# Ezreal11/EaBNet

Measured on AMD Instinct MI355X. Metric: enhanced frames/sec (16 kHz, 8-mic) at 1/2/4/8 MI355X; RTF per utterance, higher is better.
Workload: dtype f32; 1 GPU; BASELINE configs[1]/[2]: batch of 16 four-second 8-mic 16 kHz utterances per GPU, wave -> STFT+compress -> EaBNet.forward, inference, full hand-written HIP path; batch_per_gpu=16, global_batch=16, mics=8, frames_per_utt=401, freq_bins=161, parallelism=dp1 (independent shards, no collective), pipeline_depth=3

## Files before the change

### eabnet_amd/_lib.py

```python
from __future__ import annotations

import ctypes as C
import os
from typing import Optional

_HERE = os.path.dirname(os.path.abspath(__file__))
LIB_PATH = os.path.join(_HERE, "lib", "libeabnet_hip.so")
ABI_VERSION = 10
MAX_TAPS = 16
_fp = C.POINTER(C.c_float)


class TimeWindow(C.Structure):
    _fields_ = [("pos", C.c_void_p), ("count", C.c_int32), ("lens", C.c_void_p)]


class ConvDesc(C.Structure):
    _fields_ = [
        ("src0", C.c_void_p), ("src1", C.c_void_p), ("xf0", C.c_void_p), ("xf1", C.c_void_p),
        ("slope0", C.c_void_p), ("slope1", C.c_void_p),
        ("C0", C.c_int32), ("C1", C.c_int32), ("xf_mode", C.c_int32),
        ("w", C.c_void_p), ("bias", C.c_void_p),
        ("N", C.c_int32), ("Kpad", C.c_int32),
        ("B", C.c_int32), ("T", C.c_int32), ("Fin", C.c_int32), ("Fout", C.c_int32),
        ("No", C.c_int32), ("ostride", C.c_int32), ("ophase", C.c_int32), ("istride", C.c_int32),
        ("ntaps", C.c_int32), ("dt", C.c_int32 * MAX_TAPS), ("ioff", C.c_int32 * MAX_TAPS),
        ("epi", C.c_int32),
        ("aux", C.c_void_p), ("dst", C.c_void_p), ("dst_acc", C.c_void_p),
        ("Cout", C.c_int32),
        ("stats", C.c_void_p), ("nsets", C.c_int32),
        ("stat_slope0", C.c_void_p), ("stat_slope1", C.c_void_p),
        ("stat_tiles", C.c_int32), ("stat_tile0", C.c_int32), ("bm", C.c_int32),
        ("fin_stats", C.c_void_p), ("fin_gamma0", C.c_void_p), ("fin_beta0", C.c_void_p),
        ("fin_gamma1", C.c_void_p), ("fin_beta1", C.c_void_p),
        ("fin_tiles", C.c_int32), ("fin_nsets", C.c_int32), ("fin_count", C.c_int32), ("fin_eps", C.c_float),
        ("precision", C.c_int32), ("korder", C.c_int32),
        ("win", TimeWindow),
        ("fz_counter", C.c_void_p), ("fz_gamma0", C.c_void_p), ("fz_beta0", C.c_void_p), ("fz_xf0", C.c_void_p),
        ("fz_gamma1", C.c_void_p), ("fz_beta1", C.c_void_p), ("fz_xf1", C.c_void_p), ("fz_eps", C.c_float),
        ("glu_dump", C.c_void_p),
        ("ph1_w", C.c_void_p), ("ph1_No", C.c_int32), ("ph1_ophase", C.c_int32), ("ph1_ntaps", C.c_int32), ("ph1_Kpad", C.c_int32),
        ("ph1_dt", C.c_int32 * MAX_TAPS), ("ph1_ioff", C.c_int32 * MAX_TAPS),
        ("f2_w", C.c_void_p), ("f2_dst", C.c_void_p), ("f2_stats", C.c_void_p), ("f2_stat_slope0", C.c_void_p),
        ("f2_stat_slope1", C.c_void_p), ("f2_N", C.c_int32), ("f2_nsets", C.c_int32), ("f2_stat_tiles", C.c_int32),
        ("p2_mask1", C.c_int32), ("src_bf16", C.c_int32),
    ]


class WgradDesc(C.Structure):
    _fields_ = [
        ("dz", C.c_void_p), ("src0", C.c_void_p), ("src1", C.c_void_p), ("dw", C.c_void_p), ("dbias", C.c_void_p),
        ("N", C.c_int32), ("C0", C.c_int32), ("C1", C.c_int32), ("Kpad", C.c_int32),
        ("B", C.c_int32), ("T", C.c_int32), ("Fin", C.c_int32), ("Fz", C.c_int32), ("No", C.c_int32),
        ("ostride", C.c_int32), ("ophase", C.c_int32), ("istride", C.c_int32),
        ("ntaps", C.c_int32), ("dt", C.c_int32 * MAX_TAPS), ("ioff", C.c_int32 * MAX_TAPS),
        ("rows_per_wg", C.c_int32), ("precision", C.c_int32), ("bf16_mask", C.c_int32),
    ]


class Op(C.Structure):
    _fields_ = [("kind", C.c_int32), ("i", C.c_int32 * 8), ("f", C.c_float * 2), ("p", C.c_void_p * 12),
                ("win", TimeWindow), ("conv", ConvDesc), ("wgrad", WgradDesc)]


class ShiftDesc(C.Structure):
    _fields_ = [("ptr", C.c_void_p), ("row_floats", C.c_int32), ("rows", C.c_int32)]


class EabError(RuntimeError):
    pass


_SIGS = {
    "eab_abi_version": (C.c_int, []),
    "eab_error_string": (C.c_char_p, [C.c_int]),
    "eab_stft_compress_f32": (C.c_int, [C.c_void_p] * 4 + [C.c_int] * 6 + [C.c_void_p]),
    "eab_stft_compress_lens_f32": (C.c_int, [C.c_void_p] * 5 + [C.c_int] * 6 + [C.c_void_p]),
    "eab_stft_frames_f32": (C.c_int, [C.c_void_p] * 2 + [C.c_int] * 5 + [C.c_void_p]),
    "eab_filter_sum_f32": (C.c_int, [C.c_void_p] * 3 + [C.c_int] * 4 + [C.c_void_p]),
    "eab_istft_f32": (C.c_int, [C.c_void_p] * 4 + [C.c_int] * 4 + [C.c_void_p]),
    "eab_istft_lens_f32": (C.c_int, [C.c_void_p] * 5 + [C.c_int] * 4 + [C.c_void_p]),
    "eab_norm_act_win_f32": (C.c_int, [C.c_void_p] * 7 + [C.c_int] * 4 + [TimeWindow, C.c_void_p]),
    "eab_lstm64_stream_f32": (C.c_int, [C.c_void_p] * 3 + [C.c_float] + [C.c_void_p] * 4 + [C.c_int] * 4
                              + [TimeWindow, C.c_void_p]),
    "eab_bfw_filter_sum_win_f32": (C.c_int, [C.c_void_p] * 6 + [C.c_int] * 4 + [TimeWindow, C.c_void_p]),
    "eab_mlp_bfw_filter_sum_f32": (C.c_int, [C.c_void_p] * 8 + [C.c_int] * 4 + [TimeWindow, C.c_void_p]),
    "eab_zero_rows_f32": (C.c_int, [C.c_void_p] + [C.c_int] * 3 + [TimeWindow, C.c_void_p]),
    "eab_shift_rows_f32": (C.c_int, [C.c_void_p] + [C.c_int] * 5 + [C.c_void_p]),
    "eab_com_mag_mse_loss_f32": (C.c_int, [C.c_void_p] * 3 + [C.c_int] * 3 + [C.c_void_p, C.c_int, C.c_void_p, C.c_void_p,
                                            C.c_void_p]),
    "eab_energy_ratios_f32": (C.c_int, [C.c_void_p, C.c_longlong, C.c_int] * 3 + [C.c_void_p, C.c_int, C.c_void_p, C.c_int,
                                        C.c_void_p, C.c_void_p]),
    "eab_com_mag_mse_loss_lens_f32": (C.c_int, [C.c_void_p] * 3 + [C.c_int] * 4 + [C.c_void_p, C.c_int, C.c_void_p, C.c_void_p]),
    "eab_gag_pack_f32": (C.c_int, [C.c_void_p] * 4 + [C.c_int] * 4 + [TimeWindow, C.c_void_p]),
    "eab_gag_crm_f32": (C.c_int, [C.c_void_p] * 6 + [C.c_int] * 6 + [TimeWindow, C.c_void_p]),
    "eab_gag_crm_bwd_f32": (C.c_int, [C.c_void_p] * 9 + [C.c_int] * 6 + [C.c_void_p]),
    "eab_conv_tiles": (C.c_int, [C.c_int] * 3),
    "eab_conv_f32": (C.c_int, [C.POINTER(ConvDesc), C.c_void_p]),
    "eab_train_cln_bwd_f32": (C.c_int, [C.c_void_p] * 11 + [C.c_int] * 5 + [C.c_void_p]),
    "eab_conv_st_chain_plan": (C.c_int, [C.POINTER(ConvDesc), C.c_int, C.POINTER(C.c_int), C.POINTER(C.c_int), C.POINTER(C.c_int)]),
    "eab_conv_st_chain_run": (C.c_int, [C.c_void_p, C.c_void_p, C.c_int, C.c_int, C.c_int, C.c_int, C.c_void_p]),
    "eab_conv_bf16": (C.c_int, [C.POINTER(ConvDesc), C.c_void_p]),
    "eab_lstm64_bf16": (C.c_int, [C.c_void_p] * 3 + [C.c_float] + [C.c_void_p] * 3 + [C.c_int] * 3 + [C.c_void_p]),
    "eab_in_finalize_f32": (C.c_int, [C.c_void_p] + [C.c_int] * 5 + [C.c_float] + [C.c_void_p] * 6 + [C.c_void_p]),
    "eab_norm_act_f32": (C.c_int, [C.c_void_p] * 7 + [C.c_int] * 3 + [C.c_void_p]),
    "eab_lstm64_f32": (C.c_int, [C.c_void_p] * 3 + [C.c_float] + [C.c_void_p] * 3 + [C.c_int] * 3 + [C.c_void_p]),
    "eab_lstm64_prec_f32": (C.c_int, [C.c_void_p] * 3 + [C.c_float] + [C.c_void_p] * 3 + [C.c_int] * 4 + [C.c_void_p]),
    "eab_bfw_filter_sum_f32": (C.c_int, [C.c_void_p] * 6 + [C.c_int] * 4 + [C.c_void_p]),
    "eab_run_program": (C.c_int, [C.POINTER(Op), C.c_int, C.c_void_p]),
    "eab_sizeof_conv_desc": (C.c_int, []),
    "eab_sizeof_op": (C.c_int, []),
    "eab_sizeof_wgrad_desc": (C.c_int, []),
    "eab_gather_f32": (C.c_int, [C.c_void_p] * 4 + [C.c_longlong, C.c_void_p]),
    "eab_train_in_stats_f32": (C.c_int, [C.c_void_p] * 2 + [C.c_int] * 3 + [C.c_float] + [C.c_void_p] * 4 + [C.c_void_p]),
    "eab_train_in1d_f32": (C.c_int, [C.c_void_p] * 2 + [C.c_int] * 3 + [C.c_float] + [C.c_void_p] * 5 + [C.c_void_p]),
    "eab_train_in1d_multi_f32": (C.c_int, [C.c_void_p] * 2 + [C.c_int] * 4 + [C.c_float] + [C.c_void_p] * 5 + [C.c_void_p]),
    "eab_train_norm_bwd_multi_f32": (C.c_int, [C.c_void_p] * 12 + [C.c_int] * 3 + [C.c_void_p]),
    "eab_in_finalize_mr_f32": (C.c_int, [C.c_void_p] + [C.c_int] * 5 + [C.c_float] + [C.c_void_p] * 8 + [C.c_void_p]),
    "eab_train_norm_act_f32": (C.c_int, [C.c_void_p] * 5 + [C.c_int] * 4 + [C.c_void_p]),
    "eab_train_norm_bwd_f32": (C.c_int, [C.c_void_p] * 12 + [C.c_int] * 4 + [C.c_void_p]),
    "eab_glu_bwd_f32": (C.c_int, [C.c_void_p] * 3 + [C.c_longlong, C.c_int, C.c_void_p]),
    "eab_glu_bwd_ex_f32": (C.c_int, [C.c_void_p] * 3 + [C.c_longlong, C.c_int, C.c_int, C.c_void_p]),
    "eab_gate_fwd_f32": (C.c_int, [C.c_void_p] * 3 + [C.c_longlong, C.c_void_p]),
    "eab_gate_bwd_f32": (C.c_int, [C.c_void_p] * 5 + [C.c_longlong, C.c_void_p]),
    "eab_add_f32": (C.c_int, [C.c_void_p] * 3 + [C.c_longlong, C.c_void_p]),
    "eab_copy_f32": (C.c_int, [C.c_void_p] * 2 + [C.c_longlong, C.c_void_p]),
    "eab_relu_bwd_f32": (C.c_int, [C.c_void_p] * 3 + [C.c_longlong, C.c_void_p]),
    "eab_colsum_f32": (C.c_int, [C.c_void_p] * 2 + [C.c_longlong, C.c_int, C.c_void_p]),
    "eab_filter_sum_bwd_f32": (C.c_int, [C.c_void_p] * 3 + [C.c_int] * 5 + [C.c_void_p]),
    "eab_filter_sum_ld_f32": (C.c_int, [C.c_void_p] * 3 + [C.c_int] * 5 + [C.c_void_p]),
    "eab_layernorm64_fwd_f32": (C.c_int, [C.c_void_p] * 3 + [C.c_float] + [C.c_void_p] * 2 + [C.c_longlong, C.c_void_p]),
    "eab_layernorm64_bwd_f32": (C.c_int, [C.c_void_p] * 7 + [C.c_longlong, C.c_void_p]),
    "eab_lstm64_train_fwd_f32": (C.c_int, [C.c_void_p] * 5 + [C.c_int] * 3 + [C.c_void_p]),
    "eab_lstm64_bwd_f32": (C.c_int, [C.c_void_p] * 4 + [C.c_int] * 3 + [C.c_void_p]),
    "eab_lstm64_train_fwd_prec_f32": (C.c_int, [C.c_void_p] * 5 + [C.c_int] * 4 + [C.c_void_p]),
    "eab_lstm64_bwd_prec_f32": (C.c_int, [C.c_void_p] * 4 + [C.c_int] * 4 + [C.c_void_p]),
    "eab_wgrad_f32": (C.c_int, [C.POINTER(WgradDesc), C.c_void_p]),
    "eab_wgrad_batchable": (C.c_int, [C.c_void_p, C.c_int, C.c_int]),
    "eab_wgrad_batch_f32": (C.c_int, [C.c_void_p, C.c_int, C.c_int, C.c_void_p]),
    "eab_cln_stats_f32": (C.c_int, [C.c_void_p] * 2 + [C.c_int] * 4 + [C.c_float] + [C.c_void_p] * 3 + [TimeWindow, C.c_void_p]),
    "eab_cln_apply_f32": (C.c_int, [C.c_void_p] * 7 + [C.c_int] * 5 + [TimeWindow, C.c_void_p]),
    "eab_cln_step_f32": (C.c_int, [C.c_void_p] * 10 + [C.c_int] * 5 + [C.c_float, TimeWindow, C.c_void_p]),
    "eab_gate_rows_f32": (C.c_int, [C.c_void_p] * 3 + [C.c_int] * 3 + [TimeWindow, C.c_void_p]),
}
EXPORTS = tuple(_SIGS)

_lib: Optional[C.CDLL] = None


def load() -> C.CDLL:
    global _lib
    if _lib is not None:
        return _lib
    if not os.path.exists(LIB_PATH):
        raise EabError(
            f"{LIB_PATH} not found: build it with `python -c 'import __graft_entry__ as g; g.build()'` "
            "(or `make -C eabnet_amd/csrc`). eabnet_amd has no CPU fallback by design.")
    lib = C.CDLL(LIB_PATH)
    for name, (res, args) in _SIGS.items():
        try:
            fn = getattr(lib, name)
        except AttributeError as e:
            raise EabError(f"{LIB_PATH} does not export {name}") from e
        fn.restype, fn.argtypes = res, args
    if lib.eab_abi_version() != ABI_VERSION:
        raise EabError(f"ABI mismatch: library {lib.eab_abi_version()} != binding {ABI_VERSION}")
    if lib.eab_sizeof_conv_desc() != C.sizeof(ConvDesc) or lib.eab_sizeof_op() != C.sizeof(Op) \
            or lib.eab_sizeof_wgrad_desc() != C.sizeof(WgradDesc):
        raise EabError("struct layout mismatch between include/eabnet_hip.h and eabnet_amd/_lib.py")
    _lib = lib
    return lib


def check(code: int, what: str = "") -> None:
    if code != 0:
        msg = load().eab_error_string(code).decode()
        raise EabError(f"{what or 'libeabnet_hip'} failed with code {code}: {msg}")
```

### eabnet_amd/csrc/lstm.hip

```cpp
#include "common.h"
#include <cstdlib>
#include <type_traits>

#define LS_H 64
#define LS_SEQ 16
#define LS_LD (LS_H + 4)

__device__ __forceinline__ float ls_sigmoid(float x) { return __builtin_amdgcn_rcpf(1.0f + __expf(-x)); }
__device__ __forceinline__ float ls_tanh(float x) { return fmaf(2.0f, ls_sigmoid(2.0f * x), -1.0f); }

__device__ __forceinline__ float ls_row_sum(float v) {
    auto dpp = [](float x, auto ctrl) {
        return __builtin_bit_cast(float, __builtin_amdgcn_update_dpp(0, __builtin_bit_cast(int, x), decltype(ctrl)::value, 0xF, 0xF, true));
    };
    v += dpp(v, std::integral_constant<int, 0xB1>{});
    v += dpp(v, std::integral_constant<int, 0x4E>{});
    v += dpp(v, std::integral_constant<int, 0x141>{});
    v += dpp(v, std::integral_constant<int, 0x140>{});
    return v;
}

typedef unsigned int u32x4 __attribute__((ext_vector_type(4)));
#define LS_OOB 0x80000000u

template <bool LN, bool DUMP>
__global__ __launch_bounds__(256) void lstm64_kernel(const float* __restrict__ x, const float* __restrict__ ln_g,
                                                     const float* __restrict__ ln_b, float ln_eps,
                                                     const float* __restrict__ wcat, const float* __restrict__ bias,
                                                     float* __restrict__ h_out, int T, int F, int S,
                                                     const int* __restrict__ t_pos, int t_count,
                                                     float* __restrict__ c_state, float* __restrict__ gates,
                                                     const int* __restrict__ lens = nullptr) {
    __shared__ __attribute__((aligned(16))) float xs[2][LS_SEQ * LS_LD];
    __shared__ __attribute__((aligned(16))) float hs[2][LS_SEQ * LS_LD];
    const int tid = threadIdx.x, lane = tid & 63, wave = tid >> 6;
    const int ln = lane & 15, lk = lane >> 4;
    const int s0 = blockIdx.x * LS_SEQ;
    const int t_lo = t_pos ? *t_pos : 0;
    int t_hi = t_pos ? (t_lo + t_count < T ? t_lo + t_count : T) : T;
    if (lens) t_hi = min(t_hi, eab_max_len(lens, s0, LS_SEQ, S, F));

    float wx[4][16], wh[4][16];
    float bia[4];
#pragma unroll
    for (int g = 0; g < 4; ++g) {
        const int row = g * LS_H + wave * 16 + ln;
        bia[g] = bias[row];
#pragma unroll
        for (int j = 0; j < 4; ++j) {
            const f32x4 vx = *reinterpret_cast<const f32x4*>(&wcat[(size_t)row * 128 + 16 * j + 4 * lk]);
            const f32x4 vh = *reinterpret_cast<const f32x4*>(&wcat[(size_t)row * 128 + 64 + 16 * j + 4 * lk]);
#pragma unroll
            for (int s = 0; s < 4; ++s) {
                wx[g][4 * j + s] = vx[s];
                wh[g][4 * j + s] = vh[s];
            }
        }
    }

    const int ls = tid >> 4, lc = (tid & 15) * 4;
    const int sg = s0 + ls;
    const bool sv = sg < S;
    const int sb = sv ? sg / F : 0, sf = sv ? sg - sb * F : 0;
    const unsigned total_bytes = (unsigned)S * (unsigned)T * (LS_H * 4u);
    const __amdgpu_buffer_rsrc_t rx = __builtin_amdgcn_make_buffer_rsrc(const_cast<float*>(x), 0, total_bytes, 0x00020000);
    const __amdgpu_buffer_rsrc_t rh = __builtin_amdgcn_make_buffer_rsrc(h_out, 0, total_bytes, 0x00020000);
    const unsigned seq_off = (unsigned)((((size_t)sb * T * F + sf) * LS_H + lc) * 4);
    const unsigned t_stride = (unsigned)F * LS_H * 4u;
    f32x4 g4 = {1.f, 1.f, 1.f, 1.f}, b4 = {0.f, 0.f, 0.f, 0.f};
    if (LN) {
        g4 = *reinterpret_cast<const f32x4*>(ln_g + lc);
        b4 = *reinterpret_cast<const f32x4*>(ln_b + lc);
    }

    auto load_x = [&](int t) -> f32x4 {
        const unsigned off = (sv && t < t_hi) ? seq_off + (unsigned)t * t_stride : LS_OOB;
        return __builtin_bit_cast(f32x4, __builtin_amdgcn_raw_buffer_load_b128(rx, off, 0, 0));
    };
    auto norm_store = [&](f32x4 v, int buf) {
        if (LN) {
            const float mean = ls_row_sum((v[0] + v[1]) + (v[2] + v[3])) * (1.0f / 64.0f);
            f32x4 dlt = {v[0] - mean, v[1] - mean, v[2] - mean, v[3] - mean};
            const float q = ls_row_sum((dlt[0] * dlt[0] + dlt[1] * dlt[1]) + (dlt[2] * dlt[2] + dlt[3] * dlt[3]));
            const float rstd = 1.0f / sqrtf(q * (1.0f / 64.0f) + ln_eps);
#pragma unroll
            for (int j = 0; j < 4; ++j) v[j] = dlt[j] * rstd * g4[j] + b4[j];
        }
        *reinterpret_cast<f32x4*>(&xs[buf][ls * LS_LD + lc]) = v;
    };
    auto frags = [&](const float* tile, f32x4 (&a)[4]) {
        const float* arow = tile + ln * LS_LD + 4 * lk;
#pragma unroll
        for (int j = 0; j < 4; ++j) a[j] = *reinterpret_cast<const f32x4*>(arow + 16 * j);
    };
    auto mma = [&](const f32x4 (&a)[4], const float (&w)[4][16], f32x4 (&acc)[4], auto j0, auto j1) {
#pragma unroll
        for (int j = decltype(j0)::value; j < decltype(j1)::value; ++j)
#pragma unroll
            for (int s = 0; s < 4; ++s)
#pragma unroll
                for (int g = 0; g < 4; ++g)
                    acc[g] = __builtin_amdgcn_mfma_f32_16x16x4f32(a[j][s], w[g][4 * j + s], acc[g], 0, 0, 0);
    };
    using I0 = std::integral_constant<int, 0>;
    using I2 = std::integral_constant<int, 2>;
    using I4 = std::integral_constant<int, 4>;

    *reinterpret_cast<f32x4*>(&hs[0][ls * LS_LD + lc]) = __builtin_bit_cast(
        f32x4, __builtin_amdgcn_raw_buffer_load_b128(rh, (sv && t_lo > 0) ? seq_off + (unsigned)(t_lo - 1) * t_stride : LS_OOB, 0, 0));
    norm_store(load_x(t_lo), 0);
    norm_store(load_x(t_lo + 1), 1);
    const int u = wave * 16 + ln;
    float cst[4] = {0.f, 0.f, 0.f, 0.f};
    if (c_state && t_lo > 0) {
#pragma unroll
        for (int r = 0; r < 4; ++r)
            if (s0 + 4 * lk + r < S) cst[r] = c_state[(size_t)(s0 + 4 * lk + r) * LS_H + u];
    }
    __syncthreads();
    f32x4 accx[4], hf[4], xf[4];
#pragma unroll
    for (int g = 0; g < 4; ++g) accx[g] = f32x4{bia[g], bia[g], bia[g], bia[g]};
    frags(xs[0], xf);
    mma(xf, wx, accx, I0{}, I4{});
    frags(hs[0], hf);
    asm volatile("s_waitcnt lgkmcnt(0)\n\ts_barrier" ::: "memory");
    f32x4 xq = load_x(t_lo + 2), xr = load_x(t_lo + 3);

    for (int t = t_lo; t < t_hi; ++t) {
        const int cur = (t - t_lo) & 1, nxt = cur ^ 1;
        const f32x4 xn = load_x(t + 4);

        f32x4 acc[4];
#pragma unroll
        for (int g = 0; g < 4; ++g) acc[g] = accx[g];
        mma(hf, wh, acc, I0{}, I4{});
        norm_store(xq, cur);
        frags(xs[nxt], xf);
        if (LN) {
#pragma unroll
            for (int i = 0; i < 16; ++i) {
                __builtin_amdgcn_sched_group_barrier(0x008, 4, 0);
                __builtin_amdgcn_sched_group_barrier(0x002, 6, 0);
            }
        }
        __builtin_amdgcn_sched_barrier(0);

#pragma unroll
        for (int g = 0; g < 4; ++g) accx[g] = f32x4{bia[g], bia[g], bia[g], bia[g]};
        float ev[16], hval[4];
#pragma unroll
        for (int i = 0; i < 32; ++i) {
            {
                const int j = i >> 4, k = (i >> 2) & 3, g = i & 3;
                accx[g] = __builtin_amdgcn_mfma_f32_16x16x4f32(xf[j][k], wx[g][4 * j + k], accx[g], 0, 0, 0);
            }
            if (i < 8) {
#pragma unroll
                for (int n = 2 * i; n < 2 * i + 2; ++n) {
                    const float v = acc[n >> 2][n & 3];
                    ev[n] = __expf((n >> 2) == 2 ? -2.0f * v : -v);
                }
            } else if (i < 16) {
#pragma unroll
                for (int n = 2 * (i - 8); n < 2 * (i - 8) + 2; ++n) {
                    const float sg = __builtin_amdgcn_rcpf(1.0f + ev[n]);
                    ev[n] = (n >> 2) == 2 ? fmaf(2.0f, sg, -1.0f) : sg;
                }
            } else if (i < 20) {
                const int r = i - 16;
                cst[r] = fmaf(ev[4 + r], cst[r], ev[r] * ev[8 + r]);
                hval[r] = __expf(-2.0f * cst[r]);
            } else if (i < 24) {
                const int r = i - 20;
                hval[r] = ev[12 + r] * fmaf(2.0f, __builtin_amdgcn_rcpf(1.0f + hval[r]), -1.0f);
            }
            __builtin_amdgcn_sched_barrier(0);
        }

        if (DUMP) {
#pragma unroll
            for (int r = 0; r < 4; ++r) {
                const int sq = s0 + 4 * lk + r;
                if (sq < S) {
                    float* gp = gates + (((size_t)sq * T + t) * 5) * LS_H + u;
#pragma unroll
                    for (int g = 0; g < 4; ++g) gp[g * LS_H] = ev[4 * g + r];
                    gp[4 * LS_H] = cst[r];
                }
            }
        }
#pragma unroll
        for (int r = 0; r < 4; ++r) hs[nxt][(4 * lk + r) * LS_LD + u] = hval[r];
        asm volatile("s_waitcnt lgkmcnt(0)\n\ts_barrier" ::: "memory");
        frags(hs[nxt], hf);
        f32x4 hv = {0.f, 0.f, 0.f, 0.f};
        hv = *reinterpret_cast<const f32x4*>(&hs[nxt][ls * LS_LD + lc]);
        __builtin_amdgcn_sched_barrier(0);

        mma(xf, wx, accx, I2{}, I4{});
        __builtin_amdgcn_raw_buffer_store_b128(__builtin_bit_cast(u32x4, hv), rh,
                                               sv ? seq_off + (unsigned)t * t_stride : LS_OOB, 0, 0);
        xq = xr;
        xr = xn;
    }
    if (c_state) {
#pragma unroll
        for (int r = 0; r < 4; ++r)
            if (s0 + 4 * lk + r < S) c_state[(size_t)(s0 + 4 * lk + r) * LS_H + u] = cst[r];
    }
}

template <bool LN, int G, bool DUMP = false>
__global__ __launch_bounds__(256) void lstm64_q_kernel(const float* __restrict__ x, const float* __restrict__ ln_g,
                                                       const float* __restrict__ ln_b, float ln_eps,
                                                       const float* __restrict__ wcat, const float* __restrict__ bias,
                                                       float* __restrict__ h_out, int T, int F, int S,
                                                       const int* __restrict__ t_pos, int t_count,
                                                       float* __restrict__ c_state, float* __restrict__ gates = nullptr,
                                                       const int* __restrict__ lens = nullptr) {
    constexpr int NSEQ = 4 * G;
    constexpr int NCH = G == 1 ? 8 : (G == 2 ? 4 : 2);
    __shared__ __attribute__((aligned(16))) float xs[2][NSEQ * LS_LD];
    __shared__ __attribute__((aligned(16))) float hs[2][NSEQ * LS_LD];
    const int tid = threadIdx.x, lane = tid & 63, wave = tid >> 6;
    const int gate = lane & 3, u = wave * 16 + (lane >> 2);
    const int s0 = blockIdx.x * NSEQ;
    const int t_lo = t_pos ? *t_pos : 0;
    int t_hi = t_pos ? (t_lo + t_count < T ? t_lo + t_count : T) : T;
    if (lens) t_hi = min(t_hi, eab_max_len(lens, s0, NSEQ, S, F));

    float wx[64], wh[64];
    const int wrow = gate * LS_H + u;
    const float bia = bias[wrow];
#pragma unroll
    for (int k4 = 0; k4 < 16; ++k4) {
        const f32x4 vx = *reinterpret_cast<const f32x4*>(&wcat[(size_t)wrow * 128 + 4 * k4]);
        const f32x4 vh = *reinterpret_cast<const f32x4*>(&wcat[(size_t)wrow * 128 + 64 + 4 * k4]);
#pragma unroll
        for (int kk = 0; kk < 4; ++kk) {
            wx[4 * k4 + kk] = vx[kk];
            wh[4 * k4 + kk] = vh[kk];
        }
    }
    const float act_k = gate == 2 ? -2.0f : -1.0f, act_a = gate == 2 ? 2.0f : 1.0f, act_b = gate == 2 ? -1.0f : 0.0f;

    const int ls = tid >> 4, lc = (tid & 15) * 4;
    const int sg = s0 + ls;
    const bool sv = ls < NSEQ && sg < S;
    const int sb = sv ? sg / F : 0, sf = sv ? sg - sb * F : 0;
    const unsigned total_bytes = (unsigned)S * (unsigned)T * (LS_H * 4u);
    const __amdgpu_buffer_rsrc_t rx = __builtin_amdgcn_make_buffer_rsrc(const_cast<float*>(x), 0, total_bytes, 0x00020000);
    const __amdgpu_buffer_rsrc_t rh = __builtin_amdgcn_make_buffer_rsrc(h_out, 0, total_bytes, 0x00020000);
    const unsigned seq_off = (unsigned)((((size_t)sb * T * F + sf) * LS_H + lc) * 4);
    const unsigned t_stride = (unsigned)F * LS_H * 4u;
    f32x4 g4 = {1.f, 1.f, 1.f, 1.f}, b4 = {0.f, 0.f, 0.f, 0.f};
    if (LN) {
        g4 = *reinterpret_cast<const f32x4*>(ln_g + lc);
        b4 = *reinterpret_cast<const f32x4*>(ln_b + lc);
    }
    auto load_x = [&](int t) -> f32x4 {
        const unsigned off = (sv && t < t_hi) ? seq_off + (unsigned)t * t_stride : LS_OOB;
        return __builtin_bit_cast(f32x4, __builtin_amdgcn_raw_buffer_load_b128(rx, off, 0, 0));
    };
    auto norm_store = [&](f32x4 v, int buf) {
        if (LN) {
            const float mean = ls_row_sum((v[0] + v[1]) + (v[2] + v[3])) * (1.0f / 64.0f);
            f32x4 dlt = {v[0] - mean, v[1] - mean, v[2] - mean, v[3] - mean};
            const float q = ls_row_sum((dlt[0] * dlt[0] + dlt[1] * dlt[1]) + (dlt[2] * dlt[2] + dlt[3] * dlt[3]));
            const float rstd = 1.0f / sqrtf(q * (1.0f / 64.0f) + ln_eps);
#pragma unroll
            for (int j = 0; j < 4; ++j) v[j] = dlt[j] * rstd * g4[j] + b4[j];
        }
        if (ls < NSEQ) *reinterpret_cast<f32x4*>(&xs[buf][ls * LS_LD + lc]) = v;
    };
    auto quad = [](float v, auto ctrl) {
        return __builtin_bit_cast(float, __builtin_amdgcn_update_dpp(0, __builtin_bit_cast(int, v), decltype(ctrl)::value, 0xF, 0xF, true));
    };

    if (ls < NSEQ)
        *reinterpret_cast<f32x4*>(&hs[0][ls * LS_LD + lc]) = __builtin_bit_cast(
            f32x4, __builtin_amdgcn_raw_buffer_load_b128(rh, (sv && t_lo > 0) ? seq_off + (unsigned)(t_lo - 1) * t_stride : LS_OOB, 0, 0));
    norm_store(load_x(t_lo), 0);
    float cst[G][4];
#pragma unroll
    for (int q = 0; q < G; ++q)
#pragma unroll
        for (int s = 0; s < 4; ++s) {
            const int sq = s0 + 4 * q + s;
            cst[q][s] = (c_state && t_lo > 0 && sq < S) ? c_state[(size_t)sq * LS_H + u] : 0.0f;
        }
    f32x4 xq = load_x(t_lo + 1), xr = load_x(t_lo + 2);
    __syncthreads();

    for (int t = t_lo; t < t_hi; ++t) {
        const int cur = (t - t_lo) & 1, nxt = cur ^ 1;
        const f32x4 xn = load_x(t + 3);
        f32x4 acc[G][NCH];
#pragma unroll
        for (int q = 0; q < G; ++q)
#pragma unroll
            for (int c = 0; c < NCH; ++c) acc[q][c] = f32x4{0.f, 0.f, 0.f, 0.f};
#pragma unroll
        for (int part = 0; part < 2; ++part) {
            const float* src = part == 0 ? xs[cur] : hs[cur];
#pragma unroll
            for (int k4 = 0; k4 < 16; ++k4) {
#pragma unroll
                for (int q = 0; q < G; ++q) {
                    const f32x4 a = *reinterpret_cast<const f32x4*>(&src[(4 * q + gate) * LS_LD + 4 * k4]);
                    constexpr int dummy = 0;
                    (void)dummy;
                    const int c = (part * 16 + k4) % NCH;
#pragma unroll
                    for (int kk = 0; kk < 4; ++kk)
                        acc[q][c] = __builtin_amdgcn_mfma_f32_4x4x1f32(a[kk], part == 0 ? wx[4 * k4 + kk] : wh[4 * k4 + kk],
                                                                       acc[q][c], 0, 0, 0);
                }
            }
        }
        if (G == 1) {
            __builtin_amdgcn_sched_group_barrier(0x100, 6, 0);
#pragma unroll
            for (int i = 0; i < 26; ++i) {
                __builtin_amdgcn_sched_group_barrier(0x008, 4, 0);
                __builtin_amdgcn_sched_group_barrier(0x100, 1, 0);
            }
            __builtin_amdgcn_sched_group_barrier(0x008, 24, 0);
            __builtin_amdgcn_sched_barrier(0);
        }
        norm_store(xq, nxt);
#pragma unroll
        for (int q = 0; q < G; ++q) {
            f32x4 pre = acc[q][0];
#pragma unroll
            for (int c = 1; c < NCH; ++c) pre += acc[q][c];
#pragma unroll
            for (int s = 0; s < 4; ++s) {
                const float sgm = __builtin_amdgcn_rcpf(1.0f + __expf(act_k * (pre[s] + bia)));
                const float a = fmaf(act_a, sgm, act_b);
                const float gi = quad(a, std::integral_constant<int, 0x00>{}), gf = quad(a, std::integral_constant<int, 0x55>{});
                const float gg = quad(a, std::integral_constant<int, 0xAA>{}), go = quad(a, std::integral_constant<int, 0xFF>{});
                cst[q][s] = fmaf(gf, cst[q][s], gi * gg);
                const float hv = go * ls_tanh(cst[q][s]);
                if (s == gate) hs[nxt][(4 * q + s) * LS_LD + u] = hv;
                if (DUMP) {
                    const int sq = s0 + 4 * q + s;
                    if (sq < S) {
                        float* gp = gates + (((size_t)sq * T + t) * 5) * LS_H + u;
                        gp[gate * LS_H] = a;
                        if (s == gate) gp[4 * LS_H] = cst[q][s];
                    }
                }
            }
        }
        asm volatile("s_waitcnt lgkmcnt(0)\n\ts_barrier" ::: "memory");
        if (ls < NSEQ) {
            const f32x4 hv4 = *reinterpret_cast<const f32x4*>(&hs[nxt][ls * LS_LD + lc]);
            __builtin_amdgcn_raw_buffer_store_b128(__builtin_bit_cast(u32x4, hv4), rh,
                                                   sv ? seq_off + (unsigned)t * t_stride : LS_OOB, 0, 0);
        }
        xq = xr;
        xr = xn;
    }
    if (c_state && (lane & 3) == 0) {
#pragma unroll
        for (int q = 0; q < G; ++q)
#pragma unroll
            for (int s = 0; s < 4; ++s)
                if (s0 + 4 * q + s < S) c_state[(size_t)(s0 + 4 * q + s) * LS_H + u] = cst[q][s];
    }
}

template <int G>
static void lstm64_q_launch(bool ln, int grid, hipStream_t st, const float* x, const float* ln_g, const float* ln_b,
                            float ln_eps, const float* wcat, const float* bias, float* h_out, int T, int F, int S,
                            const int* t_pos, int t_count, float* cs, const int* lens) {
    if (ln)
        hipLaunchKernelGGL((lstm64_q_kernel<true, G>), dim3(grid), dim3(256), 0, st, x, ln_g, ln_b, ln_eps, wcat, bias,
                           h_out, T, F, S, t_pos, t_count, cs, nullptr, lens);
    else
        hipLaunchKernelGGL((lstm64_q_kernel<false, G>), dim3(grid), dim3(256), 0, st, x, ln_g, ln_b, ln_eps, wcat, bias,
                           h_out, T, F, S, t_pos, t_count, cs, nullptr, lens);
}

int eab_lstm64_h3_launch(const float* x, const float* ln_g, const float* ln_b, float ln_eps, const float* wcat,
                         const float* bias, float* h_out, int T, int F, int S, int precision, const int* t_pos, int t_count,
                         float* c_state, const int* lens, hipStream_t stream);

extern "C" int eab_lstm64_f32(const float* x, const float* ln_g, const float* ln_b, float ln_eps, const float* wcat,
                              const float* bias, float* h_out, int B, int T, int F, eab_stream_t stream) {
    return eab_lstm64_prec_f32(x, ln_g, ln_b, ln_eps, wcat, bias, h_out, B, T, F, EAB_PREC_F32, stream);
}

extern "C" int eab_lstm64_prec_f32(const float* x, const float* ln_g, const float* ln_b, float ln_eps,
                                   const float* wcat, const float* bias, float* h_out, int B, int T, int F,
                                   int precision, eab_stream_t stream) {
    return eab_lstm64_stream_f32(x, ln_g, ln_b, ln_eps, wcat, bias, h_out, nullptr, B, T, F, precision,
                                 eab_time_window{nullptr, 0}, stream);
}

extern "C" int eab_lstm64_stream_f32(const float* x, const float* ln_g, const float* ln_b, float ln_eps,
                                     const float* wcat, const float* bias, float* h_out, float* c_state, int B, int T,
                                     int F, int precision, eab_time_window win, eab_stream_t stream) {
    EAB_CHECK_ARG(x && wcat && bias && h_out && B > 0 && T > 0 && F > 0);
    EAB_CHECK_ARG(win.pos == nullptr || (win.count > 0 && c_state));
    EAB_CHECK_ARG(precision == EAB_PREC_F32 || precision == EAB_PREC_F16X3 || precision == EAB_PREC_BF16);
    EAB_CHECK_ARG((ln_g == nullptr) == (ln_b == nullptr));
    const long long S = (long long)B * F;
    EAB_CHECK_ARG(S * T * LS_H * 4 < (1ll << 31));
    float* cs = win.pos ? c_state : nullptr;
    if (precision != EAB_PREC_F32)
        return eab_lstm64_h3_launch(x, ln_g, ln_b, ln_eps, wcat, bias, h_out, T, F, (int)S, precision, win.pos, win.count, cs,
                                    win.lens, eab_stream(stream));
    if (S <= 2048) {
        lstm64_q_launch<1>(ln_g != nullptr, (int)((S + 3) / 4), eab_stream(stream), x, ln_g, ln_b, ln_eps, wcat, bias, h_out,
                           T, F, (int)S, win.pos, win.count, cs, win.lens);
        EAB_RETURN_LAUNCH_STATUS();
    }
    const int grid = (int)((S + LS_SEQ - 1) / LS_SEQ);
    if (ln_g)
        hipLaunchKernelGGL((lstm64_kernel<true, false>), dim3(grid), dim3(256), 0, eab_stream(stream), x, ln_g, ln_b, ln_eps,
                           wcat, bias, h_out, T, F, (int)S, win.pos, win.count, cs, nullptr, win.lens);
    else
        hipLaunchKernelGGL((lstm64_kernel<false, false>), dim3(grid), dim3(256), 0, eab_stream(stream), x, ln_g, ln_b, ln_eps,
                           wcat, bias, h_out, T, F, (int)S, win.pos, win.count, cs, nullptr, win.lens);
    EAB_RETURN_LAUNCH_STATUS();
}

int eab_lstm64_bf_train_launch(const float* x, const float* wcat, const float* bias, float* h_out, float* gates, int T, int F, int S,
                               hipStream_t stream);

extern "C" int eab_lstm64_train_fwd_f32(const float* x, const float* wcat, const float* bias, float* h_out, float* gates, int B,
                                        int T, int F, eab_stream_t stream) {
    return eab_lstm64_train_fwd_prec_f32(x, wcat, bias, h_out, gates, B, T, F, EAB_PREC_F32, stream);
}

extern "C" int eab_lstm64_train_fwd_prec_f32(const float* x, const float* wcat, const float* bias, float* h_out, float* gates, int B,
                                             int T, int F, int precision, eab_stream_t stream) {
    EAB_CHECK_ARG(x && wcat && bias && h_out && gates && B > 0 && T > 0 && F > 0);
    EAB_CHECK_ARG(precision == EAB_PREC_F32 || precision == EAB_PREC_BF16);
    const long long S = (long long)B * F;
    EAB_CHECK_ARG(S * T * LS_H * 4 < (1ll << 31));
    if (precision == EAB_PREC_BF16) return eab_lstm64_bf_train_launch(x, wcat, bias, h_out, gates, T, F, (int)S, eab_stream(stream));
    if (S <= 2048) {
        hipLaunchKernelGGL((lstm64_q_kernel<false, 1, true>), dim3((unsigned)((S + 3) / 4)), dim3(256), 0, eab_stream(stream), x,
                           nullptr, nullptr, 0.0f, wcat, bias, h_out, T, F, (int)S, nullptr, 0, nullptr, gates);
        EAB_RETURN_LAUNCH_STATUS();
    }
    const int grid = (int)((S + LS_SEQ - 1) / LS_SEQ);
    hipLaunchKernelGGL((lstm64_kernel<false, true>), dim3(grid), dim3(256), 0, eab_stream(stream), x, nullptr, nullptr, 0.0f, wcat,
                       bias, h_out, T, F, (int)S, nullptr, 0, nullptr, gates);
    EAB_RETURN_LAUNCH_STATUS();
}

extern "C" int eab_lstm64_bf16(const float* x, const float* ln_g, const float* ln_b, float ln_eps, const float* wcat,
                               const float* bias, float* h_out, int B, int T, int F, eab_stream_t stream) {
    return eab_lstm64_prec_f32(x, ln_g, ln_b, ln_eps, wcat, bias, h_out, B, T, F, EAB_PREC_BF16, stream);
}
```

### eabnet_amd/csrc/lstm_h3.hip

```cpp
#include "common.h"
#include <type_traits>

#define LH_SEQ 16
#define LH_ROW 272
#define LH_OOB 0x80000000u

typedef _Float16 h16x8 __attribute__((ext_vector_type(8)));
typedef __fp16 h16x2 __attribute__((ext_vector_type(2)));
typedef __bf16 bf16x8 __attribute__((ext_vector_type(8)));
typedef __bf16 bf16x2 __attribute__((ext_vector_type(2)));
typedef unsigned int u32x4 __attribute__((ext_vector_type(4)));

__device__ __forceinline__ float lh_sigmoid(float x) { return __builtin_amdgcn_rcpf(1.0f + __expf(-x)); }
__device__ __forceinline__ float lh_tanh(float x) { return fmaf(2.0f, lh_sigmoid(2.0f * x), -1.0f); }

__device__ __forceinline__ float lh_row_sum(float v) {
    auto dpp = [](float x, auto ctrl) {
        return __builtin_bit_cast(float, __builtin_amdgcn_update_dpp(0, __builtin_bit_cast(int, x), decltype(ctrl)::value, 0xF, 0xF, true));
    };
    v += dpp(v, std::integral_constant<int, 0xB1>{});
    v += dpp(v, std::integral_constant<int, 0x4E>{});
    v += dpp(v, std::integral_constant<int, 0x141>{});
    v += dpp(v, std::integral_constant<int, 0x140>{});
    return v;
}

template <bool BF>
__device__ __forceinline__ void lh_split2(float x0, float x1, unsigned& hi, unsigned& lo) {
    if (BF) {
        const bf16x2 h = {(__bf16)x0, (__bf16)x1};
        const bf16x2 l = {(__bf16)(x0 - (float)h[0]), (__bf16)(x1 - (float)h[1])};
        hi = __builtin_bit_cast(unsigned, h);
        lo = __builtin_bit_cast(unsigned, l);
    } else {
        const h16x2 h = __builtin_amdgcn_cvt_pkrtz(x0, x1);
        const h16x2 l = __builtin_amdgcn_cvt_pkrtz(x0 - (float)h[0], x1 - (float)h[1]);
        hi = __builtin_bit_cast(unsigned, h);
        lo = __builtin_bit_cast(unsigned, l);
    }
}

template <bool BF>
__device__ __forceinline__ float lh_join(unsigned short hi, unsigned short lo) {
    if (BF) return __builtin_bit_cast(float, (unsigned)hi << 16) + __builtin_bit_cast(float, (unsigned)lo << 16);
    return (float)__builtin_bit_cast(_Float16, hi) + (float)__builtin_bit_cast(_Float16, lo);
}

template <bool LN, bool BF, bool DUMP = false, int NS = LH_SEQ>
__global__ __launch_bounds__(256) void lstm64_h3_kernel(const float* __restrict__ x, const float* __restrict__ ln_g,
                                                        const float* __restrict__ ln_b, float ln_eps,
                                                        const float* __restrict__ wcat, const float* __restrict__ bias,
                                                        float* __restrict__ h_out, int T, int F, int S,
                                                        const int* __restrict__ t_pos, int t_count, float* __restrict__ c_state,
                                                        float* __restrict__ gates = nullptr, const int* __restrict__ lens = nullptr) {
    using v8 = std::conditional_t<BF, bf16x8, h16x8>;
    using e16 = std::conditional_t<BF, __bf16, _Float16>;
    __shared__ __attribute__((aligned(16))) char xs[2][LH_SEQ * LH_ROW];
    __shared__ __attribute__((aligned(16))) char hs[2][LH_SEQ * LH_ROW];
    const int tid = threadIdx.x, lane = tid & 63, wave = tid >> 6;
    const int ln = lane & 15, lk = lane >> 4;
    static_assert(NS == LH_SEQ || ((NS == 8 || NS == 4) && BF), "the 8- and 4-sequence forms exist for the bf16 kernel only");
    constexpr int NR = NS / 4;
    auto row_seq = [](int row) { return NS == LH_SEQ ? row : ((row & 3) < NR ? (row >> 2) * NR + (row & 3) : -1); };
    const int s0 = blockIdx.x * NS;
    const int t_lo = t_pos ? *t_pos : 0;
    int t_hi = t_pos ? (t_lo + t_count < T ? t_lo + t_count : T) : T;
    if (lens) t_hi = min(t_hi, eab_max_len(lens, s0, NS, S, F));

    v8 wxh[4][2], wxl[4][2], whh[4][2], whl[4][2];
    float bia[4];
#pragma unroll
    for (int g = 0; g < 4; ++g) {
        const int row = g * 64 + wave * 16 + ln;
        bia[g] = bias[row];
#pragma unroll
        for (int half = 0; half < 2; ++half)
#pragma unroll
            for (int kb = 0; kb < 2; ++kb) {
                const float* p = &wcat[(size_t)row * 128 + half * 64 + 32 * kb + 8 * lk];
                const f32x4 v0 = *reinterpret_cast<const f32x4*>(p), v1 = *reinterpret_cast<const f32x4*>(p + 4);
                v8 hi, lo;
#pragma unroll
                for (int j = 0; j < 8; ++j) {
                    const float w = j < 4 ? v0[j] : v1[j - 4];
                    hi[j] = (e16)w;
                    lo[j] = (e16)(w - (float)hi[j]);
                }
                if (half == 0) { wxh[g][kb] = hi; wxl[g][kb] = lo; } else { whh[g][kb] = hi; whl[g][kb] = lo; }
            }
    }

    const int ls = tid >> 4, lc = (tid & 15) * 4;
    const int sg = s0 + row_seq(ls);
    const bool sv = row_seq(ls) >= 0 && sg < S;
    const int sb = sv ? sg / F : 0, sf = sv ? sg - sb * F : 0;
    const unsigned total_bytes = (unsigned)S * (unsigned)T * 256u;
    const __amdgpu_buffer_rsrc_t rx = __builtin_amdgcn_make_buffer_rsrc(const_cast<float*>(x), 0, total_bytes, 0x00020000);
    const __amdgpu_buffer_rsrc_t rh = __builtin_amdgcn_make_buffer_rsrc(h_out, 0, total_bytes, 0x00020000);
    const unsigned seq_off = (unsigned)((((size_t)sb * T * F + sf) * 64 + lc) * 4);
    const unsigned t_stride = (unsigned)F * 256u;
    f32x4 g4 = {1.f, 1.f, 1.f, 1.f}, b4 = {0.f, 0.f, 0.f, 0.f};
    if (LN) {
        g4 = *reinterpret_cast<const f32x4*>(ln_g + lc);
        b4 = *reinterpret_cast<const f32x4*>(ln_b + lc);
    }
    const int lrow = ls * LH_ROW + (lc >> 5) * 128 + (lc & 31) * 2;

    auto load_x = [&](int t) -> f32x4 {
        const unsigned off = (sv && t < t_hi) ? seq_off + (unsigned)t * t_stride : LH_OOB;
        return __builtin_bit_cast(f32x4, __builtin_amdgcn_raw_buffer_load_b128(rx, off, 0, 0));
    };
    auto norm_store = [&](f32x4 v, int buf) {
        if (LN) {
            const float mean = lh_row_sum((v[0] + v[1]) + (v[2] + v[3])) * (1.0f / 64.0f);
            f32x4 dlt = {v[0] - mean, v[1] - mean, v[2] - mean, v[3] - mean};
            const float q = lh_row_sum((dlt[0] * dlt[0] + dlt[1] * dlt[1]) + (dlt[2] * dlt[2] + dlt[3] * dlt[3]));
            const float rstd = 1.0f / sqrtf(q * (1.0f / 64.0f) + ln_eps);
#pragma unroll
            for (int j = 0; j < 4; ++j) v[j] = dlt[j] * rstd * g4[j] + b4[j];
        }
        unsigned h01, l01, h23, l23;
        lh_split2<BF>(v[0], v[1], h01, l01);
        lh_split2<BF>(v[2], v[3], h23, l23);
        *reinterpret_cast<uint2*>(&xs[buf][lrow]) = make_uint2(h01, h23);
        if (!BF) *reinterpret_cast<uint2*>(&xs[buf][lrow + 64]) = make_uint2(l01, l23);
    };
    auto frags = [&](const char* tile, v8 (&ah)[2], v8 (&al)[2]) {
        const char* p = tile + ln * LH_ROW + lk * 16;
#pragma unroll
        for (int kb = 0; kb < 2; ++kb) {
            ah[kb] = *reinterpret_cast<const v8*>(p + kb * 128);
            if (!BF) al[kb] = *reinterpret_cast<const v8*>(p + kb * 128 + 64);
        }
    };
    auto mma = [&](const v8 (&ah)[2], const v8 (&al)[2], const v8 (&wh)[4][2], const v8 (&wl)[4][2], f32x4 (&acc)[4]) {
#pragma unroll
        for (int kb = 0; kb < 2; ++kb)
#pragma unroll
            for (int g = 0; g < 4; ++g) {
                if constexpr (BF) {
                    acc[g] = __builtin_amdgcn_mfma_f32_16x16x32_bf16(ah[kb], wh[g][kb], acc[g], 0, 0, 0);
                } else {
                    acc[g] = __builtin_amdgcn_mfma_f32_16x16x32_f16(al[kb], wh[g][kb], acc[g], 0, 0, 0);
                    acc[g] = __builtin_amdgcn_mfma_f32_16x16x32_f16(ah[kb], wl[g][kb], acc[g], 0, 0, 0);
                    acc[g] = __builtin_amdgcn_mfma_f32_16x16x32_f16(ah[kb], wh[g][kb], acc[g], 0, 0, 0);
                }
            }
    };

    for (int e = tid; e < 2 * LH_SEQ * LH_ROW / 4; e += 256) reinterpret_cast<unsigned*>(hs[0])[e] = 0u;
    __syncthreads();
    if (t_lo > 0) {
        const f32x4 hp = __builtin_bit_cast(f32x4, __builtin_amdgcn_raw_buffer_load_b128(
                                                       rh, sv ? seq_off + (unsigned)(t_lo - 1) * t_stride : LH_OOB, 0, 0));
        unsigned h01, l01, h23, l23;
        lh_split2<BF>(hp[0], hp[1], h01, l01);
        lh_split2<BF>(hp[2], hp[3], h23, l23);
        *reinterpret_cast<uint2*>(&hs[0][lrow]) = make_uint2(h01, h23);
        *reinterpret_cast<uint2*>(&hs[0][lrow + 64]) = make_uint2(l01, l23);
    }
    norm_store(load_x(t_lo), 0);
    norm_store(load_x(t_lo + 1), 1);
    const int uq = wave * 16 + ln;
    float cst[4] = {0.f, 0.f, 0.f, 0.f};
    if (c_state && t_lo > 0) {
#pragma unroll
        for (int r = 0; r < NR; ++r)
            if (s0 + row_seq(4 * lk + r) < S) cst[r] = c_state[(size_t)(s0 + row_seq(4 * lk + r)) * 64 + uq];
    }
    __syncthreads();
    f32x4 accx[4];
    v8 xh[2], xl[2], hh[2], hl[2];
#pragma unroll
    for (int g = 0; g < 4; ++g) accx[g] = f32x4{bia[g], bia[g], bia[g], bia[g]};
    frags(xs[0], xh, xl);
    mma(xh, xl, wxh, wxl, accx);
    frags(hs[0], hh, hl);
    asm volatile("s_waitcnt lgkmcnt(0)\n\ts_barrier" ::: "memory");
    f32x4 xq = load_x(t_lo + 2), xr = load_x(t_lo + 3);

    const int u = wave * 16 + ln;
    const int hcol = (u >> 5) * 128 + (u & 31) * 2;
    unsigned hdir[4];
#pragma unroll
    for (int r = 0; r < NR; ++r) {
        const int sq = s0 + row_seq(4 * lk + r);
        const int b = sq < S ? sq / F : 0, f = sq < S ? sq - b * F : 0;
        hdir[r] = sq < S ? (unsigned)((((size_t)b * T * F + f) * 64 + u) * 4) : LH_OOB;
    }
    float* gdump[4];
    if (DUMP) {
#pragma unroll
        for (int r = 0; r < NR; ++r) {
            const int sq = s0 + row_seq(4 * lk + r);
            gdump[r] = sq < S ? gates + ((size_t)sq * T * 5) * 64 + u : nullptr;
        }
    }
    for (int t = t_lo; t < t_hi; ++t) {
        const int cur = (t - t_lo) & 1, nxt = cur ^ 1;
        const f32x4 xn = load_x(t + 4);

        f32x4 acc[4];
#pragma unroll
        for (int g = 0; g < 4; ++g) acc[g] = accx[g];
        mma(hh, hl, whh, whl, acc);
        frags(xs[nxt], xh, xl);
        norm_store(xq, cur);
        __builtin_amdgcn_sched_barrier(0);
        char* hrow = &hs[nxt][hcol];
#pragma unroll
        for (int r = 0; r < NR; ++r) {
            const float ig = lh_sigmoid(acc[0][r]);
            const float fg = lh_sigmoid(acc[1][r]);
            const float gg = lh_tanh(acc[2][r]);
            const float og = lh_sigmoid(acc[3][r]);
            cst[r] = fmaf(fg, cst[r], ig * gg);
            const float h = og * lh_tanh(cst[r]);
            if (DUMP && gdump[r]) {
                float* gp = gdump[r] + (size_t)t * 320;
                gp[0] = ig;
                gp[64] = fg;
                gp[128] = gg;
                gp[192] = og;
                gp[256] = cst[r];
            }
            const e16 hi = (e16)h;
            *reinterpret_cast<e16*>(hrow + (4 * lk + r) * LH_ROW) = hi;
            if (BF) {
                __builtin_amdgcn_raw_buffer_store_b32(__builtin_bit_cast(unsigned, h), rh,
                                                      hdir[r] != LH_OOB ? hdir[r] + (unsigned)t * t_stride : LH_OOB, 0, 0);
            } else {
                const e16 lo = (e16)(h - (float)hi);
                *reinterpret_cast<e16*>(hrow + (4 * lk + r) * LH_ROW + 64) = lo;
            }
        }
        asm volatile("s_waitcnt lgkmcnt(0)\n\ts_barrier" ::: "memory");
        frags(hs[nxt], hh, hl);
        const uint2 ph = *reinterpret_cast<const uint2*>(&hs[nxt][lrow]);
        const uint2 pl = *reinterpret_cast<const uint2*>(&hs[nxt][lrow + 64]);
        __builtin_amdgcn_sched_barrier(0);

#pragma unroll
        for (int g = 0; g < 4; ++g) accx[g] = f32x4{bia[g], bia[g], bia[g], bia[g]};
        mma(xh, xl, wxh, wxl, accx);
        if (!BF) {
            const f32x4 hv = {lh_join<BF>(ph.x & 0xFFFF, pl.x & 0xFFFF), lh_join<BF>(ph.x >> 16, pl.x >> 16),
                              lh_join<BF>(ph.y & 0xFFFF, pl.y & 0xFFFF), lh_join<BF>(ph.y >> 16, pl.y >> 16)};
            __builtin_amdgcn_raw_buffer_store_b128(__builtin_bit_cast(u32x4, hv), rh,
                                                   sv ? seq_off + (unsigned)t * t_stride : LH_OOB, 0, 0);
        }
        xq = xr;
        xr = xn;
    }
    if (c_state) {
#pragma unroll
        for (int r = 0; r < NR; ++r)
            if (s0 + row_seq(4 * lk + r) < S) c_state[(size_t)(s0 + row_seq(4 * lk + r)) * 64 + u] = cst[r];
    }
}

int eab_lstm64_bf_train_launch(const float* x, const float* wcat, const float* bias, float* h_out, float* gates, int T, int F, int S,
                               hipStream_t stream) {
    if (S <= 4096)
        hipLaunchKernelGGL((lstm64_h3_kernel<false, true, true, 4>), dim3((S + 3) / 4), dim3(256), 0, stream, x, nullptr, nullptr, 0.0f,
                           wcat, bias, h_out, T, F, S, nullptr, 0, nullptr, gates);
    else
        hipLaunchKernelGGL((lstm64_h3_kernel<false, true, true>), dim3((S + LH_SEQ - 1) / LH_SEQ), dim3(256), 0, stream, x, nullptr,
                           nullptr, 0.0f, wcat, bias, h_out, T, F, S, nullptr, 0, nullptr, gates);
    EAB_RETURN_LAUNCH_STATUS();
}

int eab_lstm64_h3_launch(const float* x, const float* ln_g, const float* ln_b, float ln_eps, const float* wcat,
                         const float* bias, float* h_out, int T, int F, int S, int precision, const int* t_pos, int t_count,
                         float* c_state, const int* lens, hipStream_t stream) {
    const int grid = (S + LH_SEQ - 1) / LH_SEQ;
#define LH_GO(LN_, BF_)                                                                                                     \
    hipLaunchKernelGGL((lstm64_h3_kernel<LN_, BF_>), dim3(grid), dim3(256), 0, stream, x, ln_g, ln_b, ln_eps, wcat, bias, h_out, \
                       T, F, S, t_pos, t_count, c_state, nullptr, lens)
    if (precision == EAB_PREC_BF16) {
        if (ln_g) LH_GO(true, true); else LH_GO(false, true);
    } else {
        if (ln_g) LH_GO(true, false); else LH_GO(false, false);
    }
#undef LH_GO
    EAB_RETURN_LAUNCH_STATUS();
}
```

### eabnet_amd/csrc/program.hip

```cpp
#include "common.h"

__global__ __launch_bounds__(256) void zero_fill_kernel(float* __restrict__ p, size_t n4, size_t n) {
    const size_t i = (size_t)blockIdx.x * blockDim.x + threadIdx.x;
    const size_t stride = (size_t)gridDim.x * blockDim.x;
    for (size_t k = i; k < n4; k += stride) reinterpret_cast<f32x4*>(p)[k] = f32x4{0.f, 0.f, 0.f, 0.f};
    for (size_t k = 4 * n4 + i; k < n; k += stride) p[k] = 0.0f;
}

__global__ __launch_bounds__(256) void zero_rows_kernel(float* __restrict__ p, int T, int row4, const int* __restrict__ t_pos,
                                                        int count, long long total4) {
    const int t_lo = *t_pos;
    const long long per_b = (long long)count * row4;
    for (long long j = (long long)blockIdx.x * blockDim.x + threadIdx.x; j < total4; j += (long long)gridDim.x * blockDim.x) {
        const long long b = j / per_b, rem = j - b * per_b;
        if (t_lo + rem / row4 >= T) continue;
        reinterpret_cast<f32x4*>(p)[(b * T + t_lo) * row4 + rem] = f32x4{0.f, 0.f, 0.f, 0.f};
    }
}

extern "C" int eab_zero_rows_f32(float* ptr, int B, int T, int row_floats, eab_time_window win, eab_stream_t stream) {
    EAB_CHECK_ARG(ptr && B > 0 && T > 0 && row_floats > 0 && (row_floats % 4) == 0 && ((uintptr_t)ptr & 15) == 0);
    EAB_CHECK_ARG(win.pos == nullptr || win.count > 0);
    if (!win.pos) {
        const size_t n = (size_t)B * T * row_floats, n4 = n / 4;
        size_t g = (n4 + 255) / 256;
        if (g > 2048) g = 2048;
        hipLaunchKernelGGL(zero_fill_kernel, dim3((unsigned)g), dim3(256), 0, eab_stream(stream), ptr, n4, n);
        EAB_RETURN_LAUNCH_STATUS();
    }
    const long long total4 = (long long)B * win.count * (row_floats / 4);
    long long g = (total4 + 255) / 256;
    if (g > 2048) g = 2048;
    hipLaunchKernelGGL(zero_rows_kernel, dim3((unsigned)g), dim3(256), 0, eab_stream(stream), ptr, T, row_floats / 4, win.pos,
                       win.count, total4);
    EAB_RETURN_LAUNCH_STATUS();
}

__global__ __launch_bounds__(256) void shift_rows_kernel(const eab_shift_desc* __restrict__ descs, int T, int src_pos, int H) {
    const eab_shift_desc d = descs[blockIdx.x];
    const int h = d.rows < H ? d.rows : H;
    if (h <= 0 || d.row_floats <= 0) return;
    const size_t row = (size_t)d.row_floats, n = (size_t)h * row;
    float* base = d.ptr + (size_t)blockIdx.y * T * row;
    const float* src = base + (size_t)(src_pos - h) * row;
    float* dst = base + (size_t)(H - h) * row;
    if ((d.row_floats & 3) == 0 && ((uintptr_t)d.ptr & 15) == 0) {
        for (size_t k = threadIdx.x; k < n / 4; k += blockDim.x)
            reinterpret_cast<f32x4*>(dst)[k] = reinterpret_cast<const f32x4*>(src)[k];
    } else {
        for (size_t k = threadIdx.x; k < n; k += blockDim.x) dst[k] = src[k];
    }
}

extern "C" int eab_shift_rows_f32(const eab_shift_desc* dev_descs, int n, int B, int T, int src_pos, int H, eab_stream_t stream) {
    EAB_CHECK_ARG(dev_descs && n > 0 && B > 0 && B <= 65535 && T > 0 && H > 0);
    EAB_CHECK_ARG(src_pos <= T && (long long)src_pos >= 2ll * H);
    hipLaunchKernelGGL(shift_rows_kernel, dim3((unsigned)n, (unsigned)B), dim3(256), 0, eab_stream(stream), dev_descs, T, src_pos, H);
    EAB_RETURN_LAUNCH_STATUS();
}

extern "C" int eab_abi_version(void) { return EAB_ABI_VERSION; }

extern "C" const char* eab_error_string(int code) {
    if (code == EAB_OK) return "ok";
    if (code == EAB_EINVAL) return "invalid argument (shape, limit or null pointer) -- nothing was launched";
    if (code == EAB_EUNSUPPORTED) return "configuration not built into libeabnet_hip";
    if (code >= EAB_EHIP_BASE) return hipGetErrorString((hipError_t)(code - EAB_EHIP_BASE));
    return "unknown eabnet_hip error";
}

extern "C" int eab_run_program(const eab_op* ops, int n_ops, eab_stream_t stream) {
    EAB_CHECK_ARG(ops && n_ops >= 0);
    for (int k = 0; k < n_ops; ++k) {
        const eab_op& o = ops[k];
        int rc;
        switch (o.kind) {
            case EAB_OP_CONV:
                rc = eab_conv_f32(&o.conv, stream);
                break;
            case EAB_OP_CONV_CHAIN:
                rc = eab_conv_st_chain_run((const eab_conv_desc*)o.p[0], (const int*)o.p[1], o.i[0], o.i[1], o.i[2], o.i[3], stream);
                break;
            case EAB_OP_IN_FINALIZE:
                rc = eab_in_finalize_mr_f32((const float*)o.p[0], o.i[0], o.i[1], o.i[2], o.i[3], o.i[4], o.f[0],
                                            (const float*)o.p[1], (const float*)o.p[2], (float*)o.p[3],
                                            (const float*)o.p[4], (const float*)o.p[5], (float*)o.p[6], (float*)o.p[7],
                                            (float*)o.p[8], stream);
                break;
            case EAB_OP_NORM_ACT:
                if (o.win.pos || o.win.lens)
                    rc = o.i[3] > 0 && o.i[1] % o.i[3] == 0
                             ? eab_norm_act_win_f32((const float*)o.p[0], (const float*)o.p[1], (const float*)o.p[2],
                                                    (const float*)o.p[3], (const float*)o.p[4], (const float*)o.p[5],
                                                    (float*)o.p[6], o.i[0], o.i[3], o.i[1] / o.i[3], o.i[2], o.win, stream)
                             : EAB_EINVAL;
                else
                    rc = eab_norm_act_f32((const float*)o.p[0], (const float*)o.p[1], (const float*)o.p[2],
                                          (const float*)o.p[3], (const float*)o.p[4], (const float*)o.p[5],
                                          (float*)o.p[6], o.i[0], o.i[1], o.i[2], stream);
                break;
            case EAB_OP_LSTM64:
                rc = eab_lstm64_stream_f32((const float*)o.p[0], (const float*)o.p[1], (const float*)o.p[2], o.f[0],
                                           (const float*)o.p[3], (const float*)o.p[4], (float*)o.p[5], (float*)o.p[6],
                                           o.i[0], o.i[1], o.i[2], o.i[3], o.win, stream);
                break;
            case EAB_OP_BFW_FS:
                rc = eab_mlp_bfw_filter_sum_f32((const float*)o.p[0], (const float*)o.p[6], (const float*)o.p[7],
                                                (const float*)o.p[1], (const float*)o.p[2], (const float*)o.p[3],
                                                (float*)o.p[4], (float*)o.p[5], o.i[0], o.i[1], o.i[2], o.i[3], o.win,
                                                stream);
                break;
            case EAB_OP_MEMSET0: {
                if (o.win.pos) {
                    rc = eab_zero_rows_f32((float*)const_cast<void*>(o.p[0]), o.i[2], o.i[3], o.i[4], o.win, stream);
                    break;
                }
                const size_t bytes = ((size_t)(uint32_t)o.i[1] << 32) | (uint32_t)o.i[0];
                if (!o.p[0] || (bytes & 3) || ((uintptr_t)o.p[0] & 15)) {
                    rc = EAB_EINVAL;
                    break;
                }
                const size_t n = bytes / 4, n4 = n / 4;
                size_t g = (n4 + 255) / 256;
                if (g > 2048) g = 2048;
                if (g == 0) g = 1;
                hipLaunchKernelGGL(zero_fill_kernel, dim3((unsigned)g), dim3(256), 0, eab_stream(stream),
                                   (float*)const_cast<void*>(o.p[0]), n4, n);
                rc = eab_hip_status(hipGetLastError());
                break;
            }
            case EAB_OP_GAG_PACK:
                rc = eab_gag_pack_f32((const float*)o.p[0], (const float*)o.p[1], (float*)o.p[2], (float*)o.p[3], o.i[0],
                                      o.i[1], o.i[2], o.i[3], o.win, stream);
                break;
            case EAB_OP_GAG_CRM:
                rc = eab_gag_crm_f32((const float*)o.p[0], (const float*)o.p[1], (const float*)o.p[2],
                                     (const float*)o.p[3], (float*)o.p[4], (float*)o.p[5], o.i[0], o.i[1], o.i[2], o.i[3],
                                     o.i[4], o.i[5], o.win, stream);
                break;
#define EAB_P(k) ((const float*)o.p[k])
#define EAB_W(k) ((float*)const_cast<void*>(o.p[k]))
#define EAB_N64(k) ((long long)(((unsigned long long)(uint32_t)o.i[(k) + 1] << 32) | (uint32_t)o.i[k]))
            case EAB_OP_GATHER:
                rc = eab_gather_f32(EAB_P(0), (const int32_t*)o.p[1], (const int32_t*)o.p[2], EAB_W(3), EAB_N64(0), stream);
                break;
            case EAB_OP_IN_STATS:
                rc = o.p[6] && o.i[3] > 0
                         ? eab_train_in1d_multi_f32(EAB_P(0), EAB_P(1), o.i[0], o.i[1], o.i[2], o.i[3], o.f[0], EAB_P(2), EAB_P(3),
                                                    EAB_W(4), EAB_W(5), EAB_W(6), stream)
                     : o.p[6] ? eab_train_in1d_f32(EAB_P(0), EAB_P(1), o.i[0], o.i[1], o.i[2], o.f[0], EAB_P(2), EAB_P(3), EAB_W(4),
                                                 EAB_W(5), EAB_W(6), stream)
                            : eab_train_in_stats_f32(EAB_P(0), EAB_P(1), o.i[0], o.i[1], o.i[2], o.f[0], EAB_P(2), EAB_P(3),
                                                     EAB_W(4), EAB_W(5), stream);
                break;
            case EAB_OP_TR_NORM_ACT:
                rc = eab_train_norm_act_f32(EAB_P(0), EAB_P(1), EAB_P(2), EAB_P(3), EAB_W(4), o.i[0], o.i[1], o.i[2], o.i[3],
                                            stream);
                break;
            case EAB_OP_NORM_BWD:
                rc = o.i[4] > 0 ? eab_train_norm_bwd_multi_f32(EAB_P(0), EAB_P(4), EAB_P(1), EAB_P(2), EAB_P(3), EAB_P(5), EAB_W(6),
                                                               EAB_P(7), EAB_W(8), EAB_W(9), EAB_W(10), EAB_W(11), o.i[0], o.i[1],
                                                               o.i[4], stream)
                                : eab_train_norm_bwd_f32(EAB_P(0), EAB_P(1), EAB_P(2), EAB_P(3), EAB_P(4), EAB_P(5), EAB_W(6), EAB_P(7),
                                                         EAB_W(8), EAB_W(9), EAB_W(10), EAB_W(11), o.i[0], o.i[1], o.i[2], o.i[3],
                                                         stream);
                break;
            case EAB_OP_GLU_BWD:
                rc = eab_glu_bwd_ex_f32(EAB_P(0), EAB_P(1), EAB_W(2), EAB_N64(0), o.i[2], o.i[3], stream);
                break;
            case EAB_OP_GATE_FWD:
                rc = eab_gate_fwd_f32(EAB_P(0), EAB_P(1), EAB_W(2), EAB_N64(0), stream);
                break;
            case EAB_OP_GATE_BWD:
                rc = eab_gate_bwd_f32(EAB_P(0), EAB_P(1), EAB_P(2), EAB_W(3), EAB_W(4), EAB_N64(0), stream);
                break;
            case EAB_OP_ADD:
                rc = eab_add_f32(EAB_P(0), EAB_P(1), EAB_W(2), EAB_N64(0), stream);
                break;
            case EAB_OP_RELU_BWD:
                rc = eab_relu_bwd_f32(EAB_P(0), EAB_P(1), EAB_W(2), EAB_N64(0), stream);
                break;
            case EAB_OP_COLSUM:
                rc = eab_colsum_f32(EAB_P(0), EAB_W(1), EAB_N64(0), o.i[2], stream);
                break;
            case EAB_OP_FILTER_SUM:
                rc = eab_filter_sum_ld_f32(EAB_P(0), EAB_P(1), EAB_W(2), o.i[0], o.i[1], o.i[2], o.i[3], o.i[4], stream);
                break;
            case EAB_OP_FS_BWD:
                rc = eab_filter_sum_bwd_f32(EAB_P(0), EAB_P(1), EAB_W(2), o.i[0], o.i[1], o.i[2], o.i[3], o.i[4], stream);
                break;
            case EAB_OP_LN_FWD:
                rc = eab_layernorm64_fwd_f32(EAB_P(0), EAB_P(1), EAB_P(2), o.f[0], EAB_W(3), EAB_W(4), EAB_N64(0), stream);
                break;
            case EAB_OP_LN_BWD:
                rc = eab_layernorm64_bwd_f32(EAB_P(0), EAB_P(1), EAB_P(2), EAB_P(3), EAB_W(4), EAB_W(5), EAB_W(6), EAB_N64(0),
                                             stream);
                break;
            case EAB_OP_LSTM_TRAIN:
                rc = eab_lstm64_train_fwd_prec_f32(EAB_P(0), EAB_P(1), EAB_P(2), EAB_W(3), EAB_W(4), o.i[0], o.i[1], o.i[2], o.i[3], stream);
                break;
            case EAB_OP_LSTM_BWD:
                rc = eab_lstm64_bwd_prec_f32(EAB_P(0), EAB_P(1), EAB_P(2), EAB_W(3), o.i[0], o.i[1], o.i[2], o.i[3], stream);
                break;
            case EAB_OP_GAG_CRM_BWD:
                rc = eab_gag_crm_bwd_f32(EAB_P(0), EAB_P(1), EAB_P(2), EAB_P(3), EAB_P(4), EAB_W(5), EAB_W(6), EAB_W(7), EAB_W(8), o.i[0],
                                         o.i[1], o.i[2], o.i[3], o.i[4], o.i[5], stream);
                break;
            case EAB_OP_WGRAD: {
                int run = 1;
                while (k + run < n_ops && ops[k + run].kind == EAB_OP_WGRAD) ++run;
                const int nb = eab_wgrad_batchable(&o.wgrad, run, (int)sizeof(eab_op));
                rc = eab_wgrad_batch_f32(&o.wgrad, nb, (int)sizeof(eab_op), stream);
                k += nb - 1;
                break;
            }
            case EAB_OP_CLN_STATS:
                rc = eab_cln_stats_f32(EAB_P(0), EAB_P(1), o.i[0], o.i[1], o.i[2], o.i[3], o.f[0], (double*)const_cast<void*>(o.p[2]),
                                       (double*)const_cast<void*>(o.p[3]), EAB_W(4), o.win, stream);
                break;
            case EAB_OP_CLN_APPLY:
                rc = eab_cln_apply_f32(EAB_P(0), EAB_P(1), EAB_P(2), EAB_P(3), EAB_P(4), EAB_P(5), EAB_W(6), o.i[0], o.i[1], o.i[2],
                                       o.i[3], o.i[4], o.win, stream);
                break;
            case EAB_OP_CLN_STEP:
                rc = eab_cln_step_f32(EAB_P(0), EAB_P(1), (double*)const_cast<void*>(o.p[2]), (double*)const_cast<void*>(o.p[3]),
                                      EAB_W(4), EAB_P(5), EAB_P(6), EAB_P(7), EAB_P(8), EAB_W(9), o.i[0], o.i[1], o.i[2], o.i[3],
                                      o.i[4], o.f[0], o.win, stream);
                break;
            case EAB_OP_CLN_BWD:
                rc = eab_train_cln_bwd_f32(EAB_P(0), EAB_P(1), EAB_P(2), EAB_P(3), EAB_P(4), EAB_P(5), (double*)const_cast<void*>(o.p[6]),
                                           EAB_W(7), EAB_W(8), EAB_P(9), EAB_W(10), o.i[0], o.i[1], o.i[2], o.i[3], o.i[4], stream);
                break;
            case EAB_OP_GATE_ROWS:
                rc = eab_gate_rows_f32(EAB_P(0), EAB_P(1), EAB_W(2), o.i[0], o.i[1], o.i[2], o.win, stream);
                break;
#undef EAB_P
#undef EAB_W
#undef EAB_N64
            default:
                rc = EAB_EINVAL;
        }
        if (rc != EAB_OK) return rc;
    }
    return EAB_OK;
}

extern "C" int eab_sizeof_conv_desc(void) { return (int)sizeof(eab_conv_desc); }
extern "C" int eab_sizeof_op(void) { return (int)sizeof(eab_op); }
extern "C" int eab_sizeof_wgrad_desc(void) { return (int)sizeof(eab_wgrad_desc); }
```

### eabnet_amd/model.py

```python
from __future__ import annotations

import ctypes as C
import math
import os
from collections import OrderedDict
from typing import Dict, Optional, Tuple

import numpy as np
import torch
import torch.nn as nn

from . import _lib
from . import program as prg
from .graphs import LaneGraphs
from .runtime import BoundProgram, chain_planner, chain_tables, encode, fuse_step
from .runtime import graph_branches_allowed
from .spec import GagConfig, NetConfig, ParamSpec, gag_param_specs, param_specs


class _Scope(nn.Module):
    """Anonymous container: only exists so that ``state_dict()`` produces the
    dotted keys of the reference's module tree."""


def _default_init(spec: ParamSpec) -> torch.Tensor:
    t = torch.empty(spec.shape, dtype=torch.float32)
    k = spec.kind
    if k in ("conv_w", "convT_w", "lin_w", "bias", "lstm"):
        a = 1.0 / math.sqrt(max(spec.fan_in, 1))
        return t.uniform_(-a, a)
    if k in ("norm_w", "ln_w"):
        return t.fill_(1.0)
    if k in ("norm_b", "ln_b"):
        return t.zero_()
    if k == "prelu":
        return t.fill_(0.25)
    if k == "bn_mean":
        return t.zero_()
    if k == "bn_var":
        return t.fill_(1.0)
    if k == "bn_count":
        return torch.zeros((), dtype=torch.long)
    raise ValueError(k)


def _attach(root: nn.Module, dotted: str, p: torch.Tensor) -> None:
    node = root
    parts = dotted.split(".")
    for name in parts[:-1]:
        child = node._modules.get(name)
        if child is None:
            child = _Scope()
            node.add_module(name, child)
        node = child
    if isinstance(p, nn.Parameter):
        node.register_parameter(parts[-1], p)
    else:
        node.register_buffer(parts[-1], p)


class _Bound(BoundProgram):
    BOUNDARY = ("in", "out", "in2")

    def __init__(self, prog: prg.Program, device: torch.device):
        self.prog = prog
        self.weights = torch.from_numpy(prog.weights).to(device)
        self.acts = torch.empty(max(prog.act_floats, 1), dtype=torch.float32, device=device)
        super().__init__(device, {"w": self.weights, "a": self.acts}, {"run": prog.ops}, {"run": prog.lanes}, {"run": prog.sync})
        self.ops = self.arrays["run"]
        self.reset_counters()
        self.t_pos = torch.zeros(1, dtype=torch.int32, device=device) if prog.chunk else None
        self.lens = torch.full((prog.B,), prog.T, dtype=torch.int32, device=device) if prog.varlen else None
        self.window = {"t_pos": self.t_pos.data_ptr() if prog.chunk else None, "chunk": prog.chunk,
                       "lens": self.lens.data_ptr() if prog.varlen else None}
        self.fused, self.exec_ops = None, None
        self._carry_dev = None

    def reset_counters(self) -> None:
        for ref, n in self.prog.zero_init:
            self.acts[ref.off:ref.off + n].zero_()

    def __del__(self):
        try:
            if torch.cuda.is_available():
                torch.cuda.synchronize(self.device)
        except Exception:
            pass

    @property
    def graph(self) -> Optional[LaneGraphs]:
        return self.graphs["run"] if self.graphs else None

    static_in = property(lambda self: self.static.get("in"))
    static_out = property(lambda self: self.static.get("out"))
    static_in2 = property(lambda self: self.static.get("in2"))

    def update_weights(self, flat: np.ndarray) -> None:
        self.weights.copy_(torch.from_numpy(flat), non_blocking=False)

    def bind(self, in_ptr: int, out_ptr: int, in2_ptr: Optional[int] = None) -> bool:
        if not super().bind(in_ptr, out_ptr, in2_ptr):
            return False
        self._carry_dev = None
        p = self.prog
        if not p.chunk:
            return True
        self.fused, self.exec_ops = None, None
        self.arenas.pop("chain", None)
        fused = fuse_step(p.ops, p.chunk, os.environ.get("EAB_ST_CHAIN", "1") != "0", os.environ.get("EAB_CLN_STEP", "1") != "0",
                          chain_planner(self.ops))
        if len(fused) < len(p.ops):
            tables = chain_tables(self.ops, fused)
            if tables:
                self.arenas["chain"] = torch.frombuffer(bytearray(tables), dtype=torch.uint8).to(self.device)
            self.fused = fused
            self.exec_ops = encode([op for op, _, _ in fused], self.bases(), **self.window)
        return True

    @property
    def chains(self) -> list:
        return [(first, count) for op, first, count in (self.fused or []) if op.kind == prg.OP_CONV_CHAIN]

    @property
    def n_exec(self) -> int:
        return len(self.exec_ops) if self.exec_ops is not None else 0

    def upload_carry(self) -> None:
        if self._carry_dev is not None or not self.prog.carry:
            return
        bases = self.bases()
        descs = (_lib.ShiftDesc * len(self.prog.carry))()
        for d, (ref, row, rows) in zip(descs, self.prog.carry):
            d.ptr, d.row_floats, d.rows = bases[ref.arena] + 4 * ref.off, row, rows
        self._carry_dev = torch.frombuffer(bytearray(bytes(descs)), dtype=torch.uint8).to(self.device)

    def rebase(self, src_pos: int, stream: int) -> int:
        p = self.prog
        if not (p.chunk and 2 * p.history <= src_pos <= p.T):
            raise ValueError(f"rebase at position {src_pos} of a window of {p.T} frames with history {p.history}")
        self.upload_carry()
        if p.carry:
            _lib.check(_lib.load().eab_shift_rows_f32(self._carry_dev.data_ptr(), len(p.carry), p.B, p.T, src_pos, p.history,
                                                      C.c_void_p(stream)), "eab_shift_rows_f32")
        return p.history

    def buffers(self, use_graph: bool, in_shape, out_shape, in2_shape=None):
        if use_graph and self.capture(in_shape, out_shape, in2_shape):
            return (self.static_in, self.static_out, self.static_in2), self.graph.replay
        bufs = tuple(None if s is None else torch.zeros(s, dtype=torch.float32, device=self.device)
                     for s in (in_shape, out_shape, in2_shape))
        self.bind(*(None if b is None else b.data_ptr() for b in bufs))
        return bufs, lambda: self.run(torch.cuda.current_stream().cuda_stream)

    def _launch(self, name: str, stream: int, first: int, n: int) -> None:
        if first == 0 and n == len(self.prog.ops) and self.exec_ops is not None:
            _lib.check(_lib.load().eab_run_program(self.exec_ops, self.n_exec, C.c_void_p(stream)), "eab_run_program")
            return
        super()._launch(name, stream, first, n)

    def run(self, stream: int, first: int = 0, count: Optional[int] = None) -> None:
        super().run("run", stream, first, count)

    def view(self, act: prg.Act) -> torch.Tensor:
        p = self.prog
        n = p.B * p.T * act.F * act.C
        assert act.ref.arena == "a"
        return self.acts[act.ref.off:act.ref.off + n].view(p.B, p.T, act.F, act.C)


AUTO_BUCKETS = tuple(64 << k for k in range(8))


def bucket_for(T: int, caps) -> Optional[int]:
    for c in caps:
        if c >= T:
            return int(c)
    return None


def check_lengths(lengths, B: int, T: int, lo: int = 1, unit: str = "the call's frame count", integral: bool = False):
    if isinstance(lengths, torch.Tensor):
        if lengths.dtype.is_floating_point or lengths.dtype == torch.bool or lengths.is_complex():
            raise ValueError(f"lengths must be integers, got {lengths.dtype}")
        if tuple(lengths.shape) != (B,):
            raise ValueError(f"lengths must have shape ({B},), got {tuple(lengths.shape)}")
        if lengths.is_cuda:
            return lengths
        vals = [int(v) for v in lengths.tolist()]
    else:
        vals = list(lengths)
        if integral and any(isinstance(v, bool) or not isinstance(v, (int, float, np.integer, np.floating)) or int(v) != v
                            for v in vals):
            raise ValueError(f"lengths must be integers, got {vals[:4]}")
        vals = [int(v) for v in vals]
        if len(vals) != B:
            raise ValueError(f"lengths must hold {B} values (one per utterance), got {len(vals)}")
    bad = [v for v in vals if not lo <= v <= T]
    if bad:
        raise ValueError(f"lengths must lie in [{lo}, {T}] ({unit}), got {bad[:4]}")
    return vals


def _device_lengths(lens, device: torch.device) -> torch.Tensor:
    if isinstance(lens, torch.Tensor):
        return lens.to(device=device, dtype=torch.int32, non_blocking=True).contiguous()
    return torch.as_tensor(lens, dtype=torch.int32).pin_memory().to(device, non_blocking=True)


def _refuse_differentiable(module: nn.Module, what: str, reason: str):
    return NotImplementedError(
        f"{type(module).__name__}: {what} ({reason}).  eabnet_amd runs differentiable calls on its HIP training programs "
        "(eabnet_amd/train.py, train_gag.py) and has no operator fallback; call under torch.no_grad() for inference.")


class _HipModule(nn.Module):

    def _init_params(self, specs) -> None:
        self._specs = specs
        for key, spec in specs.items():
            t = _default_init(spec)
            _attach(self, key, t if spec.is_buffer else nn.Parameter(t))
        self._bound: "OrderedDict[tuple, _Bound]" = OrderedDict()
        self._packed_version: Dict[tuple, tuple] = {}
        self.dump_bfw = False
        self.use_graph = True
        self.precision = "f32"
        self.training_backend = None
        self.length_buckets = None
        self.max_resident_programs = 8
        self.max_resident_bytes = 8 << 30
        self._varlen_bound: "OrderedDict[tuple, _Bound]" = OrderedDict()
        self._varlen_version: Dict[tuple, tuple] = {}

    def _param_fingerprint(self) -> tuple:
        slots = self.__dict__.get("_slot_list")
        if slots is None:
            slots = []
            for mod in self.modules():
                slots += [(mod._parameters, n) for n in mod._parameters] + [(mod._buffers, n) for n in mod._buffers]
            self.__dict__["_slot_list"] = slots
        fp = []
        for d, n in slots:
            t = d[n]
            fp.append((t.data_ptr(), t._version))
        return tuple(fp)

    def _numpy_params(self) -> Dict[str, np.ndarray]:
        sd = self.state_dict()
        return {k: sd[k].detach().to("cpu", torch.float32).numpy() for k, s in self._specs.items()
                if s.kind != "bn_count"}

    def _program(self, B: int, T: int, F: int, device: torch.device, varlen: bool = False, fit: bool = False) -> Optional[_Bound]:
        chains = bool(self.__dict__.get("parallel_chains", True))
        key = (B, T, F, str(device), self.precision, chains)
        cache, versions = (self._varlen_bound, self._varlen_version) if varlen else (self._bound, self._packed_version)
        limit, budget = (self.max_resident_programs, self.max_resident_bytes) if varlen else (1, math.inf)
        fp = self._param_fingerprint()
        bound = cache.get(key)
        stale = bound is None or ("bf_w" in bound.prog.taps) != self.dump_bfw
        if stale or versions.get(key) != fp:
            prog = prg.lower(self.cfg, self._numpy_params(), B, T, F, dump_bfw=self.dump_bfw, precision=self.precision,
                             parallel_chains=chains, varlen=varlen)
            if stale:
                need = 4 * max(prog.act_floats, 1)
                if fit and need > budget:
                    return None
                while cache and (len(cache) >= limit or sum(4 * b.acts.numel() for b in cache.values()) + need > budget):
                    old, _ = cache.popitem(last=False)
                    versions.pop(old, None)
                bound = cache[key] = _Bound(prog, device)
            else:
                bound.update_weights(prog.weights)
            versions[key] = fp
        cache.move_to_end(key)
        return bound

    def _bucket_caps(self) -> Tuple[int, ...]:
        lb = self.length_buckets
        if lb is None:
            return ()
        if isinstance(lb, str):
            if lb != "auto":
                raise ValueError(f"length_buckets must be None, 'auto' or an ascending tuple of frame counts, got {lb!r}")
            return AUTO_BUCKETS
        caps = tuple(int(c) for c in lb)
        if not caps or any(c < 1 for c in caps) or any(b <= a for a, b in zip(caps, caps[1:])):
            raise ValueError(f"length_buckets must be an ascending tuple of positive frame counts, got {lb!r}")
        return caps

    def _varlen_call(self, T: int, B: int, lengths, needs_graph: bool) -> Optional[Tuple[int, object]]:
        if lengths is None:
            if self.length_buckets is None or not self.cfg.is_causal or needs_graph or self.dump_bfw:
                return None
            cap = bucket_for(T, self._bucket_caps())
            return None if cap is None else (cap, T)
        lens = check_lengths(lengths, B, T)
        if needs_graph:
            raise _refuse_differentiable(self, "lengths= under autograd (or BatchNorm in train mode)",
                                         "per-utterance lengths are an inference form; training with lengths (masked batch "
                                         "statistics, gradients) is not implemented")
        if not self.cfg.is_causal:
            raise NotImplementedError(f"{type(self).__name__}: lengths= needs is_causal=True -- the non-causal S-TCM taps of "
                                      "the last frames of an utterance read the frames after it, so a padded batch cannot "
                                      "reproduce the one-at-a-time result")
        if self.dump_bfw:
            raise NotImplementedError(f"{type(self).__name__}: lengths= with dump_bfw (a test hook of the exact-shape path)")
        cap = bucket_for(T, self._bucket_caps()) if self.length_buckets is not None else None
        return (cap if cap is not None else T), lens

    def varlen_arena_bytes(self) -> Dict[tuple, int]:
        return {k: 4 * b.acts.numel() for k, b in self._varlen_bound.items()}

    def _forward(self, inputs: tuple, out_shape: tuple, tax: int, lengths) -> torch.Tensor:
        x0, name = inputs[0], type(self).__name__
        noun = "input" if len(inputs) == 1 else "inputs"
        B, T, F = x0.shape[0], x0.shape[tax], x0.shape[tax + 1]
        needs_graph = self._needs_graph(*inputs)
        vl = self._varlen_call(T, B, lengths, needs_graph)
        if needs_graph:
            from . import train
            if not (all(x.is_cuda for x in inputs) and next(self.parameters()).is_cuda):
                raise _lib.EabError(f"eabnet_amd.{name} trains on MI355X only: move the {noun} and the module to 'cuda'. "
                                    "There is no CPU fallback by design.")
            if any(x.requires_grad for x in inputs):
                raise _refuse_differentiable(self, *self._input_grad_refusal)
            if self.norm_type == "BN" and not self.training:
                raise _refuse_differentiable(self, "BatchNorm in eval mode under autograd", "the training programs implement "
                                             "BatchNorm's train mode; call .train(), or torch.no_grad() for inference")
            lower = self._training_lowering()
            self.training_backend = "hip"
            xs = tuple(x.detach().to(torch.float32).contiguous() for x in inputs)
            return train.forward_train(self, xs, lower)
        if not all(x.is_cuda for x in inputs):
            raise _lib.EabError(f"eabnet_amd.{name} inference runs on MI355X only: move the {noun} (and module) to "
                                "'cuda'. There is no CPU fallback by design.")
        _lib.load()
        xs = tuple(x.detach().to(torch.float32) for x in inputs)
        use_graph = self.use_graph and not self.dump_bfw and not torch.cuda.is_current_stream_capturing()
        with torch.cuda.device(x0.device):
            if vl is None:
                xs = tuple(x.contiguous() for x in xs)
                bound = self._program(B, T, F, x0.device)
                if use_graph and bound.capture(xs[0].shape, out_shape, xs[1].shape if len(xs) > 1 else None):
                    for buf, x in zip((bound.static_in, bound.static_in2), xs):
                        buf.copy_(x, non_blocking=True)
                    bound.graph.replay()
                    out = bound.static_out.clone()
                else:
                    out = torch.empty(out_shape, dtype=torch.float32, device=x0.device)
                    bound.bind(xs[0].data_ptr(), out.data_ptr(), xs[1].data_ptr() if len(xs) > 1 else None)
                    bound.run(torch.cuda.current_stream().cuda_stream)
            else:
                T_cap, lens = vl
                bound = self._program(B, T_cap, F, x0.device, varlen=True)
                if isinstance(lens, int):
                    bound.lens.fill_(lens)
                elif isinstance(lens, torch.Tensor) and lens.is_cuda:
                    bound.lens.copy_(lens.to(torch.int32), non_blocking=True)
                else:
                    bound.lens.copy_(torch.as_tensor(lens, dtype=torch.int32).pin_memory(), non_blocking=True)
                pad = lambda shp, ax: tuple(shp[:ax]) + (T_cap,) + tuple(shp[ax + 1:])
                (b_in, b_out, b_in2), launch = bound.buffers(use_graph, pad(xs[0].shape, tax), pad(out_shape, -2),
                                                             pad(xs[1].shape, tax) if len(xs) > 1 else None)
                for buf, x in zip((b_in, b_in2), xs):
                    buf.narrow(tax, 0, T).copy_(x, non_blocking=True)
                launch()
                out = b_out[..., :T, :].clone()
                self._last_varlen = (b_in, b_out, b_in2)
        self._last = (bound, *xs)
        return out

    def stream_begin(self, B: int, T_max: int, chunk: int = 1, F: int = 161, device=None, endless: bool = False) -> EaBNetStream:
        if self.training:
            raise RuntimeError("stream_begin: call .eval() first (BatchNorm must use its running statistics)")
        _lib.load()
        device = torch.device(device) if device is not None else next(self.parameters()).device
        if device.type != "cuda":
            raise _lib.EabError("streaming inference runs on MI355X only: move the module to 'cuda'")
        if chunk < 1 or T_max < 1:
            raise ValueError("chunk and T_max must be positive")
        with torch.cuda.device(device):
            prog = prg.lower(self.cfg, self._numpy_params(), B, T_max, F, precision=self.precision, chunk=chunk)
            if endless and T_max < prog.min_window:
                raise ValueError(f"endless stream: a window of T_max={T_max} frames is too small, this network reads "
                                 f"{prog.history} frames back and needs at least {prog.min_window} "
                                 f"(2 * {prog.history} + chunk)")
            return EaBNetStream(self, _Bound(prog, device), B, T_max, F, chunk, endless)

    def _needs_graph(self, *inputs) -> bool:
        needs = torch.is_grad_enabled() and (any(x.requires_grad for x in inputs)
                                             or any(p.requires_grad for p in self.parameters()))
        return needs or (self.norm_type == "BN" and self.training)


class EaBNet(_HipModule):

    def __init__(self, k1: tuple = (2, 3), k2: tuple = (1, 3), c: int = 64, M: int = 9, embed_dim: int = 64,
                 kd1: int = 5, cd1: int = 64, d_feat: int = 256, p: int = 6, q: int = 3, is_causal: bool = True,
                 is_u2: bool = True, bf_type: str = "lstm", topo_type: str = "mimo", intra_connect: str = "cat",
                 norm_type: str = "IN"):
        super().__init__()
        self.k1, self.k2, self.c, self.M, self.embed_dim = tuple(k1), tuple(k2), c, M, embed_dim
        self.kd1, self.cd1, self.d_feat, self.p, self.q = kd1, cd1, d_feat, p, q
        self.is_causal, self.is_u2, self.bf_type = is_causal, is_u2, bf_type
        self.topo_type, self.intra_connect, self.norm_type = topo_type, intra_connect, norm_type
        self.cfg = NetConfig(k1=tuple(k1), k2=tuple(k2), c=c, M=M, embed_dim=embed_dim, kd1=kd1, cd1=cd1,
                             d_feat=d_feat, p=p, q=q, is_causal=is_causal, is_u2=is_u2, bf_type=bf_type,
                             topo_type=topo_type, intra_connect=intra_connect, norm_type=norm_type)
        self._init_params(param_specs(self.cfg))

    def forward(self, inpt: torch.Tensor, lengths=None) -> torch.Tensor:
        if inpt.ndim == 4:
            inpt = inpt.unsqueeze(-2)
        if inpt.ndim != 5 or inpt.shape[-1] != 2 or inpt.shape[-2] != self.M:
            raise ValueError(f"expected (B,T,F,{self.M},2), got {tuple(inpt.shape)}")
        out = self._forward((inpt,), (inpt.shape[0], 2, inpt.shape[1], inpt.shape[2]), 1, lengths)
        if self.topo_type == "miso":
            out = out.sum(dim=-1)
        return out.to(inpt.dtype)

    _input_grad_refusal = ("the input requires grad", "the training programs produce parameter gradients only, as the "
                           "reference's training loop needs")

    def _training_lowering(self):
        from . import train
        if not train.supported(self.cfg):
            raise _refuse_differentiable(self, "topology outside the training programs", train.unsupported_reason(self.cfg))
        return train.lower_train


class EaBNetStream:

    def __init__(self, net, bound: _Bound, B: int, T_max: int, F: int, chunk: int, endless: bool = False):
        self.net, self.bound, self.B, self.T_max, self.F, self.chunk = net, bound, B, T_max, F, chunk
        self.endless = endless
        self.pos = 0
        self._closed = False
        self.post = isinstance(net, GaGNet)
        if self.post:
            in_shape, out_shape, in2_shape = (B, 2, T_max, F), (net.q, B, 2, T_max, F), (B, 2, T_max, F)
        else:
            in_shape, out_shape, in2_shape = (B, T_max, F, net.M, 2), (B, 2, T_max, F), None
        (self._in, self._out, self._in2), self._launch = bound.buffers(net.use_graph, in_shape, out_shape, in2_shape)
        if endless:
            assert T_max >= bound.prog.min_window
            bound.upload_carry()

    @property
    def history(self) -> int:
        return self.bound.prog.history

    def reset(self) -> None:
        self.pos, self._closed = 0, False

    def step(self, x: torch.Tensor, pre_x: Optional[torch.Tensor] = None):
        tdim = 2 if self.post else 1
        n = x.shape[tdim]
        if self._closed:
            raise RuntimeError("the previous step was a short final chunk: call reset() before the next utterance")
        want = (self.B, 2, n, self.F) if self.post else (self.B, n, self.F, self.net.M, 2)
        if tuple(x.shape) != want or not 0 < n <= self.chunk or (self.post and (pre_x is None or pre_x.shape != x.shape)):
            raise ValueError(f"expected {want} with n <= {self.chunk}, got {tuple(x.shape)}")
        if not self.endless and self.pos + n > self.T_max:
            raise ValueError(f"utterance longer than the T_max={self.T_max} given to stream_begin")
        if not x.is_cuda:
            raise _lib.EabError("stream.step needs CUDA (ROCm) tensors; there is no CPU fallback by design.")
        if self.endless and self.pos + self.chunk > self.T_max:
            with torch.cuda.device(x.device):
                self.pos = self.bound.rebase(self.pos, torch.cuda.current_stream().cuda_stream)
        lo, hi, end = self.pos, self.pos + n, self.pos + self.chunk
        with torch.cuda.device(x.device), torch.no_grad():
            for buf, src in ((self._in, x), (self._in2, pre_x)):
                if buf is None:
                    continue
                buf.narrow(tdim, lo, n).copy_(src, non_blocking=True)
                if n < self.chunk and end > hi:
                    buf.narrow(tdim, hi, min(end, self.T_max) - hi).zero_()
            self.bound.t_pos.fill_(lo)
            self._launch()
            out = self._out[..., lo:hi, :].clone()
        self.pos += n
        self._closed = n < self.chunk
        if self.post:
            out = out.to(x.dtype)
            return [out[j].permute(0, 1, 3, 2) for j in range(self.net.q)]
        if self.net.topo_type == "miso":
            out = out.sum(dim=-1)
        return out.to(x.dtype)


def _replica(module: nn.Module) -> nn.Module:
    import copy
    rep = copy.copy(module)
    rep._modules = {k: (_replica(v) if v is not None else None) for k, v in module._modules.items()}
    if isinstance(rep, _HipModule):
        rep._bound, rep._packed_version = OrderedDict(), {}
        rep.length_buckets, rep._varlen_bound, rep._varlen_version = None, OrderedDict(), {}
        rep.__dict__.pop("_slot_list", None)
    return rep


_PIPE_STREAMS: Dict[tuple, list] = {}


def _sync_knobs(src: nn.Module, rep: nn.Module) -> None:
    for k in ("precision", "use_graph", "training"):
        if k in src.__dict__:
            rep.__dict__[k] = src.__dict__[k]
    for name, child in src._modules.items():
        if child is not None:
            _sync_knobs(child, rep._modules[name])


class Pipeline:

    def __init__(self, model: nn.Module, depth: int = 2, front_end: Optional[tuple] = None, prepare=None):
        if depth < 1:
            raise ValueError("depth must be >= 1")
        if front_end is not None and prepare is not None:
            raise ValueError("front_end and prepare are alternatives")
        self.model, self.depth, self.front_end, self.prepare = model, depth, front_end, prepare
        self._replicas = [_replica(model) for _ in range(depth)] if depth > 1 else [model]
        if depth > 1:
            for rep in self._replicas:
                for m in rep.modules():
                    if isinstance(m, GaGNet):
                        m.parallel_chains = False
        self._streams: list = []
        self._pending: list = []
        self._n = 0

    @property
    def outstanding(self) -> int:
        return len(self._pending)

    @staticmethod
    def _tensors(obj):
        if torch.is_tensor(obj):
            yield obj
        elif isinstance(obj, dict):
            for v in obj.values():
                yield from Pipeline._tensors(v)
        elif isinstance(obj, (list, tuple)):
            for v in obj:
                yield from Pipeline._tensors(v)

    def submit(self, *inputs: torch.Tensor) -> None:
        if self.outstanding >= self.depth:
            raise RuntimeError("collect() a result before submitting more than `depth` batches")
        if not inputs:
            raise ValueError("nothing to submit")
        takes_host = self.front_end is not None or self.prepare is not None
        if not takes_host and not all(x.is_cuda for x in inputs):
            raise _lib.EabError("Pipeline.submit needs CUDA (ROCm) tensors (host waves only with front_end= / prepare=); "
                                "there is no CPU fallback by design.")
        dev_in = next((x.device for x in inputs if x.is_cuda), None)
        device = dev_in if dev_in is not None else next(self.model.parameters()).device
        if device.type != "cuda":
            raise _lib.EabError("Pipeline runs on MI355X only: move the module to 'cuda'. There is no CPU fallback by design.")
        with torch.cuda.device(device):
            if not self._streams:
                key = (str(device), self.depth)
                if key not in _PIPE_STREAMS:
                    from .graphs import overlapping_streams
                    _PIPE_STREAMS[key] = overlapping_streams(device, self.depth)
                self._streams = _PIPE_STREAMS[key]
            if takes_host and not all(x.is_cuda for x in inputs):
                _stager(device).run_beside(self._streams)
            slot = self._n % self.depth
            self._n += 1
            st = self._streams[slot]
            st.wait_stream(torch.cuda.current_stream())
            extra = None
# ... 555 lines not shown
```

### eabnet_amd/program.py

```python
from __future__ import annotations

import os
from dataclasses import dataclass, field
from typing import Dict, List, Optional, Sequence, Tuple

import numpy as np

from ._lib import MAX_TAPS
from .spec import GagConfig, NetConfig, gag_param_specs, gate_key, param_specs, unet_decoder_layers, unet_encoder_layers

XF_NONE, XF_NORM_PRELU, XF_PRELU_NORM = 0, 1, 2
EPI_LINEAR, EPI_GLU, EPI_RELU, EPI_MULSIG, EPI_ADD, EPI_DUALGATE, EPI_PHASE2 = 0, 1, 2, 3, 4, 5, 6
OP_CONV, OP_IN_FINALIZE, OP_NORM_ACT, OP_LSTM64, OP_BFW_FS, OP_MEMSET0, OP_GAG_PACK, OP_GAG_CRM = 1, 2, 3, 4, 5, 6, 7, 8
OP_CONV_CHAIN = 9
(OP_GATHER, OP_IN_STATS, OP_TR_NORM_ACT, OP_NORM_BWD, OP_GLU_BWD, OP_GATE_FWD, OP_GATE_BWD, OP_ADD, OP_RELU_BWD, OP_COLSUM,
 OP_FILTER_SUM, OP_FS_BWD, OP_LN_FWD, OP_LN_BWD, OP_LSTM_TRAIN, OP_LSTM_BWD) = range(16, 32)
OP_WGRAD = 32
OP_CLN_STATS, OP_CLN_APPLY, OP_GATE_ROWS = 33, 34, 35
OP_GAG_CRM_BWD, OP_CLN_BWD = 36, 37
OP_CLN_STEP = 38
NB_SUMS_ZEROED = 0x100
NB_SUM_COPIES = 8
STORE_BF16 = 0x200
ACT_SIGMOID, ACT_TANH, ACT_RELU = 0, 1, 2
GAG_PRE_LD = 324
GAG_LIN_LD = 192
PREC_F32, PREC_F16X3, PREC_BF16 = 0, 1, 2
PREC_CODE = {"f32": PREC_F32, "f16x3": PREC_F16X3, "bf16": PREC_BF16}
KORDER_TAP, KORDER_CHUNK, KORDER_FRAG = 0, 1, 2
ST_GLU_KMAX = 512
PATCH_MAX = 352
EPS_IN = 1e-5
EPS_LN = 1e-5
ALIGN = 64
CUS = 256


@dataclass(frozen=True)
class Ref:
    arena: str
    off: int = 0


@dataclass
class Act:
    ref: Ref
    F: int
    C: int
    xf: Optional[Ref] = None
    slope: Optional[Ref] = None
    mode: int = XF_NONE
    raw: bool = False


@dataclass
class ConvOp:
    src0: Ref
    src1: Optional[Ref]
    xf0: Optional[Ref]
    xf1: Optional[Ref]
    slope0: Optional[Ref]
    slope1: Optional[Ref]
    C0: int
    C1: int
    xf_mode: int
    w: Ref
    bias: Optional[Ref]
    N: int
    Kpad: int
    B: int
    T: int
    Fin: int
    Fout: int
    No: int
    ostride: int
    ophase: int
    istride: int
    dt: List[int]
    ioff: List[int]
    epi: int
    aux: Optional[Ref]
    dst: Ref
    dst_acc: Optional[Ref]
    Cout: int
    stats: Optional[Ref]
    nsets: int
    stat_slope0: Optional[Ref]
    stat_slope1: Optional[Ref]
    stat_tiles: int
    stat_tile0: int
    bm: int
    fin_stats: Optional[Ref] = None
    fin_gamma0: Optional[Ref] = None
    fin_beta0: Optional[Ref] = None
    fin_gamma1: Optional[Ref] = None
    fin_beta1: Optional[Ref] = None
    fin_tiles: int = 0
    fin_nsets: int = 0
    fin_count: int = 0
    fin_eps: float = 0.0
    precision: int = PREC_F32
    korder: int = KORDER_TAP
    win: bool = False
    name: str = ""
    kind: int = OP_CONV
    fz_counter: Optional[Ref] = None
    fz_gamma0: Optional[Ref] = None
    fz_beta0: Optional[Ref] = None
    fz_xf0: Optional[Ref] = None
    fz_gamma1: Optional[Ref] = None
    fz_beta1: Optional[Ref] = None
    fz_xf1: Optional[Ref] = None
    fz_eps: float = 0.0
    ph1_w: Optional[Ref] = None
    ph1_No: int = 0
    ph1_ophase: int = 0
    ph1_Kpad: int = 0
    ph1_dt: List[int] = field(default_factory=list)
    ph1_ioff: List[int] = field(default_factory=list)
    f2_w: Optional[Ref] = None
    f2_dst: Optional[Ref] = None
    f2_stats: Optional[Ref] = None
    f2_stat_slope0: Optional[Ref] = None
    f2_stat_slope1: Optional[Ref] = None
    f2_N: int = 0
    f2_nsets: int = 0
    f2_stat_tiles: int = 0
    p2_mask1: int = 0
    glu_dump: Optional[Ref] = None
    src_bf16: int = 0


@dataclass
class FinalizeOp:
    stats: Ref
    B: int
    C: int
    nsets: int
    stat_tiles: int
    count: int
    eps: float
    gamma0: Ref
    beta0: Ref
    xf0: Ref
    gamma1: Optional[Ref] = None
    beta1: Optional[Ref] = None
    xf1: Optional[Ref] = None
    mr0: Optional[Ref] = None
    name: str = ""
    kind: int = OP_IN_FINALIZE


@dataclass
class NormActOp:
    a: Ref
    xfa: Ref
    slopea: Ref
    b: Optional[Ref]
    xfb: Optional[Ref]
    slopeb: Optional[Ref]
    out: Ref
    B: int
    P: int
    C: int
    T: int = 0
    win: bool = False
    name: str = ""
    kind: int = OP_NORM_ACT


@dataclass
class LstmOp:
    x: Ref
    ln_g: Optional[Ref]
    ln_b: Optional[Ref]
    ln_eps: float
    wcat: Ref
    bias: Ref
    h_out: Ref
    B: int
    T: int
    F: int
    precision: int = PREC_F32
    c_state: Optional[Ref] = None
    win: bool = False
    name: str = ""
    kind: int = OP_LSTM64


@dataclass
class BfwOp:
    y1: Ref
    w2: Ref
    b2: Ref
    x: Ref
    out: Ref
    bfw: Optional[Ref]
    B: int
    T: int
    F: int
    M: int
    w1: Optional[Ref] = None
    b1: Optional[Ref] = None
    win: bool = False
    name: str = ""
    kind: int = OP_BFW_FS


@dataclass
class MemsetOp:
    ptr: Ref
    nfloats: int
    B: int = 0
    T: int = 0
    row: int = 0
    win: bool = False
    name: str = ""
    kind: int = OP_MEMSET0


@dataclass
class GagPackOp:
    inpt: Ref
    pre_x: Ref
    enc_in: Ref
    pre: Ref
    B: int
    T: int
    F: int
    pre_ld: int = GAG_PRE_LD
    win: bool = False
    name: str = ""
    kind: int = OP_GAG_PACK


@dataclass
class GagCrmOp:
    pre: Ref
    g: Ref
    r: Ref
    i: Ref
    pre_out: Ref
    planar: Ref
    B: int
    T: int
    F: int
    act: int
    pre_ld: int = GAG_PRE_LD
    win: bool = False
    name: str = ""
    kind: int = OP_GAG_CRM


@dataclass
class ClnStatsOp:
    x: Ref
    slope: Optional[Ref]
    sums: Ref
    state: Optional[Ref]
    mr: Ref
    B: int
    T: int
    P: int
    C: int
    eps: float
    win: bool = False
    name: str = ""
    kind: int = OP_CLN_STATS


@dataclass
class ClnApplyOp:
    x: Ref
    mr: Ref
    gain: Ref
    bias: Ref
    slope: Ref
    add: Optional[Ref]
    out: Ref
    B: int
    T: int
    P: int
    C: int
    mode: int
    win: bool = False
    name: str = ""
    kind: int = OP_CLN_APPLY


@dataclass
class ClnStepOp:
    x: Ref
    stat_slope: Optional[Ref]
    sums: Ref
    state: Ref
    mr: Ref
    gain: Ref
    bias: Ref
    slope: Ref
    add: Optional[Ref]
    out: Ref
    B: int
    T: int
    P: int
    C: int
    mode: int
    eps: float
    win: bool = True
    name: str = ""
    kind: int = OP_CLN_STEP


@dataclass
class ConvChainOp:
    descs: Ref
    codes: Ref
    n: int
    B: int
    lds_bytes: int
    bf16: int
    plan: Tuple[int, ...] = ()
    name: str = ""
    kind: int = OP_CONV_CHAIN


@dataclass
class GateRowsOp:
    a: Ref
    r: Ref
    z: Ref
    B: int
    T: int
    row: int
    win: bool = False
    name: str = ""
    kind: int = OP_GATE_ROWS


def conv_tiles(T: int, No: int, bm: int) -> int:
    return (T * No + bm - 1) // bm


def patch_positions(bm: int, No: int, Fin: int, istride: int, dt, ioff) -> int:
    dt_min, io_min, io_max = min(0, min(dt)), min(0, min(ioff)), max(0, max(ioff))
    hi_need = (No - 1) * istride + io_max - (Fin - 1)
    Fp = Fin - io_min + max(hi_need, 0)
    return ((bm - 1) // No + 2 - dt_min) * Fp


def glu_row_order(N: int) -> np.ndarray:
    r = np.arange(N)
    return (r % 64 // 32) * (N // 2) + (r // 64) * 32 + r % 32


def pack_taps(w_nck: np.ndarray, taps_k: Sequence[int]) -> np.ndarray:
    N, C, _ = w_nck.shape
    upt = (C + 15) // 16
    out = np.zeros((N, len(taps_k), upt * 16), dtype=np.float32)
    for j, k in enumerate(taps_k):
        out[:, j, :C] = w_nck[:, :, k]
    return out.reshape(N, -1)


def pack_f16x3(wp: np.ndarray) -> np.ndarray:
    N, K = wp.shape
    assert K % 4 == 0
    if np.abs(wp).max(initial=0.0) >= 65504.0:
        raise ValueError("f16x3 precision needs |weight| < 65504")
    hi = wp.astype(np.float16)
    lo = (wp - hi.astype(np.float32)).astype(np.float16)
    out = np.empty((N, K // 4, 8), dtype=np.float16)
    out[:, :, :4] = hi.reshape(N, K // 4, 4)
    out[:, :, 4:] = lo.reshape(N, K // 4, 4)
    return np.ascontiguousarray(out).view(np.float32).reshape(N, K)


def _frag_index(N: int, K: int):
    nb, m2, lane, j = np.meshgrid(np.arange(N // 16), np.arange(K // 16), np.arange(64), np.arange(4), indexing="ij")
    return nb * 16 + (lane & 15), 16 * m2 + 8 * (j >> 1) + 2 * (lane >> 4) + (j & 1)


def frag_row_order(N: int, dual: bool) -> np.ndarray:
    r = np.arange(N)
    if not dual:
        return r
    return ((r // 16) % 2) * (N // 2) + (r // 32) * 16 + r % 16


def pack_frag(wp: np.ndarray, dual: bool = False) -> np.ndarray:
    N, K = wp.shape
    assert N % 16 == 0 and K % 16 == 0
    n, k = _frag_index(N, K)
    return np.ascontiguousarray(wp[frag_row_order(N, dual)][n, k],
                                dtype=wp.dtype if np.issubdtype(wp.dtype, np.integer) else np.float32).reshape(-1)


def unpack_frag(flat: np.ndarray, N: int, K: int, dual: bool = False) -> np.ndarray:
    n, k = _frag_index(N, K)
    w = np.empty((N, K), np.float32)
    w[n, k] = np.asarray(flat, np.float32).reshape(n.shape)
    out = np.empty_like(w)
    out[frag_row_order(N, dual)] = w
    return out


class WeightArena:

    def __init__(self):
        self.chunks: List[np.ndarray] = []
        self.chunks_by_name: Dict[str, np.ndarray] = {}
        self.size = 0
        self.index: Dict[str, Ref] = {}

    def add(self, name: str, arr: np.ndarray) -> Ref:
        if name in self.index:
            return self.index[name]
        flat = np.ascontiguousarray(arr, dtype=np.float32).reshape(-1)
        pad = (-flat.size) % ALIGN
        ref = Ref("w", self.size)
        self.chunks.append(flat)
        self.chunks_by_name[name] = flat
        if pad:
            self.chunks.append(np.zeros(pad, dtype=np.float32))
        self.size += flat.size + pad
        self.index[name] = ref
        return ref

    def flat(self) -> np.ndarray:
        return np.concatenate(self.chunks) if self.chunks else np.zeros(0, np.float32)


@dataclass
class Program:
    cfg: object
    B: int
    T: int
    F: int
    ops: list
    weights: np.ndarray
    act_floats: int
    taps: Dict[str, Act]
    flops: int = 0
    lanes: List[int] = field(default_factory=list)
    sync: Dict[int, list] = field(default_factory=dict)
    chunk: int = 0
    zero_init: List[Tuple[Ref, int]] = field(default_factory=list)
    varlen: bool = False
    carry: List[Tuple[Ref, int, int]] = field(default_factory=list)
    history: int = 0

    @property
    def min_window(self) -> int:
        return 2 * self.history + self.chunk


def carry_table(ops: Sequence, chunk: int) -> Tuple[List[Tuple[Ref, int, int]], int]:
    reach: Dict[Ref, List[int]] = {}

    def need(ref: Optional[Ref], row: int, rows: int) -> None:
        if ref is None or rows <= 0:
            return
        e = reach.setdefault(ref, [row, 0])
        assert e[0] == row, f"{ref}: read with {row} and {e[0]} floats per time row"
        e[1] = max(e[1], rows)
    for op in ops:
        if op.kind == OP_CONV:
            back = max([0] + [-d for d in list(op.dt) + list(op.ph1_dt)])
            need(op.src0, op.Fin * op.C0, back)
            need(op.src1, op.Fin * op.C1, back)
        elif op.kind == OP_LSTM64:
            need(op.h_out, op.F * 64, 1)
    far = max([1] + [e[1] for e in reach.values()])
    return [(ref, e[0], e[1]) for ref, e in reach.items()], -(-far // chunk) * chunk


class Lowering:
    spec_fn = staticmethod(param_specs)

    def __init__(self, cfg, params: Dict[str, np.ndarray], B: int, T: int, F: int = 161,
                 dump_bfw: bool = False, precision: str = "f32", chunk: int = 0):
        cfg.check_supported()
        self.chunk = chunk
        if chunk:
            if cfg.norm_type not in ("BN", "cLN") or not cfg.is_causal:
                raise NotImplementedError("streaming needs norm_type='BN' (eval) or 'cLN' and is_causal=True: InstanceNorm "
                                          "statistics and centred S-TCM taps look at the whole utterance")
            if precision == "f16x3":
                raise NotImplementedError("streaming runs in 'f32' or 'bf16' (BASELINE config 5); 'f16x3' is an offline mode")
        if precision not in ("f32", "f16x3", "bf16"):
            raise ValueError(f"precision must be 'f32', 'f16x3' or 'bf16', got {precision!r}")
# ... 746 lines not shown
```

### eabnet_amd/runtime.py

```python
from __future__ import annotations

import ctypes as C
import functools
import os
import warnings
from typing import Callable, Dict, List, Mapping, Optional, Sequence, Tuple

import torch

from . import _lib
from . import program as prg
from .graphs import LaneGraphs, plan_segments, single_lane

_CONV_PTRS = ("src0", "src1", "xf0", "xf1", "slope0", "slope1", "w", "bias", "aux", "dst", "dst_acc", "stats", "stat_slope0",
              "stat_slope1", "fin_stats", "fin_gamma0", "fin_beta0", "fin_gamma1", "fin_beta1", "fz_counter", "fz_gamma0",
              "fz_beta0", "fz_xf0", "fz_gamma1", "fz_beta1", "fz_xf1", "glu_dump", "ph1_w", "f2_w", "f2_dst", "f2_stats",
              "f2_stat_slope0", "f2_stat_slope1")
_CONV_INTS = ("C0", "C1", "xf_mode", "N", "Kpad", "B", "T", "Fin", "Fout", "No", "ostride", "ophase", "istride", "epi", "Cout",
              "nsets", "stat_tiles", "stat_tile0", "bm", "fin_tiles", "fin_nsets", "fin_count", "precision", "korder",
              "p2_mask1", "src_bf16", "ph1_No", "ph1_ophase", "ph1_Kpad", "f2_N", "f2_nsets", "f2_stat_tiles")
_CONV_FLOATS = ("fin_eps", "fz_eps")
_WGRAD_PTRS = ("dz", "src0", "src1", "dw", "dbias")
_WGRAD_INTS = ("N", "C0", "C1", "Kpad", "B", "T", "Fin", "Fz", "No", "ostride", "ophase", "istride", "precision", "bf16_mask")
_LAYOUT = {
    prg.FinalizeOp: (("B", "C", "nsets", "stat_tiles", "count"),
                     ("stats", "gamma0", "beta0", "xf0", "gamma1", "beta1", "xf1", "mr0"), ("eps",)),
    prg.NormActOp: (("B", "P", "C", "T"), ("a", "xfa", "slopea", "b", "xfb", "slopeb", "out"), ()),
    prg.LstmOp: (("B", "T", "F", "precision"), ("x", "ln_g", "ln_b", "wcat", "bias", "h_out", "c_state"), ("ln_eps",)),
    prg.BfwOp: (("B", "T", "F", "M"), ("y1", "w2", "b2", "x", "out", "bfw", "w1", "b1"), ()),
    prg.MemsetOp: ((None, None, "B", "T", "row"), ("ptr",), ()),
    prg.ClnStatsOp: (("B", "T", "P", "C"), ("x", "slope", "sums", "state", "mr"), ("eps",)),
    prg.ClnApplyOp: (("B", "T", "P", "C", "mode"), ("x", "mr", "gain", "bias", "slope", "add", "out"), ()),
    prg.GateRowsOp: (("B", "T", "row"), ("a", "r", "z"), ()),
    prg.GagPackOp: (("B", "T", "F", "pre_ld"), ("inpt", "pre_x", "enc_in", "pre"), ()),
    prg.GagCrmOp: (("B", "T", "F", "pre_ld", prg.GAG_LIN_LD, "act"), ("pre", "g", "r", "i", "pre_out", "planar"), ()),
    prg.ClnStepOp: (("B", "T", "P", "C", "mode"),
                    ("x", "stat_slope", "sums", "state", "mr", "gain", "bias", "slope", "add", "out"), ("eps",)),
    prg.ConvChainOp: (("n", "B", "lds_bytes", "bf16"), ("descs", "codes"), ()),
}


def _i32(v) -> int:
    return C.c_int32(int(v) & 0xFFFFFFFF).value


def _taps(dt, ioff, n: int, dst_dt, dst_ioff) -> None:
    for j in range(n):
        dst_dt[j] = dt[j] if j < len(dt) else 0
        dst_ioff[j] = ioff[j] if j < len(ioff) else 0


def encode(ops: Sequence, bases: Mapping[str, Optional[int]], t_pos: Optional[int] = None, chunk: int = 0,
           lens: Optional[int] = None, out=None):
    arr = (_lib.Op * len(ops))() if out is None else out

    def A(r):
        return None if r is None else bases[r.arena] + 4 * r.off
    for o, op in zip(arr, ops):
        o.kind = op.kind
        win = o.conv.win if op.kind == prg.OP_CONV else o.win
        if getattr(op, "win", False):
            win.pos, win.count = t_pos, chunk
        if lens is not None and hasattr(op, "win"):
            win.lens = lens
        if op.kind == prg.OP_CONV:
            d = o.conv
            for f in _CONV_PTRS:
                setattr(d, f, A(getattr(op, f)))
            for f in _CONV_INTS:
                setattr(d, f, int(getattr(op, f)))
            for f in _CONV_FLOATS:
                setattr(d, f, float(getattr(op, f)))
            d.ntaps, d.ph1_ntaps = len(op.dt), len(op.ph1_dt)
            _taps(op.dt, op.ioff, _lib.MAX_TAPS, d.dt, d.ioff)
            _taps(op.ph1_dt, op.ph1_ioff, _lib.MAX_TAPS, d.ph1_dt, d.ph1_ioff)
        elif op.kind == prg.OP_WGRAD:
            d = o.wgrad
            for f in _WGRAD_PTRS:
                setattr(d, f, A(getattr(op, f)))
            for f in _WGRAD_INTS:
                setattr(d, f, int(getattr(op, f)))
            d.ntaps = len(op.dt)
            _taps(op.dt, op.ioff, _lib.MAX_TAPS, d.dt, d.ioff)
        else:
            layout = _LAYOUT.get(type(op))
            if layout is None:
                ints, ptrs, flts = op.i, op.p, op.f
            else:
                ints = [a if a is None or isinstance(a, int) else getattr(op, a) for a in layout[0]]
                ptrs = [getattr(op, a) for a in layout[1]]
                flts = [getattr(op, a) for a in layout[2]]
                if op.kind == prg.OP_MEMSET0:
                    nbytes = 4 * op.nfloats
                    ints[0:2] = [nbytes & 0xFFFFFFFF, nbytes >> 32]
            for j, v in enumerate(ints):
                o.i[j] = _i32(v)
            for j, r in enumerate(ptrs):
                o.p[j] = A(r)
            for j, v in enumerate(flts):
                o.f[j] = float(v)
    return arr


def _aligned(nfloats: int) -> int:
    return nfloats + (-nfloats) % prg.ALIGN


def fuse_step(ops: Sequence, chunk: int, chain: bool, cln_step: bool,
              plan_chain: Callable[[int, int], Optional[Tuple[Sequence[int], int, int]]]) -> List[Tuple[object, int, int]]:
    n = len(ops)
    single = [plan_chain(k, 1) if chain and chunk and op.kind == prg.OP_CONV and op.korder == prg.KORDER_FRAG else None
              for k, op in enumerate(ops)]

    def cln_pair(k: int) -> bool:
        a, b = ops[k], ops[k + 1] if k + 1 < n else None
        return (cln_step and chunk == 1 and b is not None and a.kind == prg.OP_CLN_STATS and b.kind == prg.OP_CLN_APPLY
                and a.x == b.x and a.mr == b.mr and (a.B, a.T, a.P, a.C) == (b.B, b.T, b.P, b.C) and a.win and b.win
                and a.state is not None)
    fused, k, table = [], 0, 0
    while k < n:
        j = k
        while j < n and single[j] is not None and single[j][2] == single[k][2]:
            j += 1
        got = plan_chain(k, j - k) if j - k >= 2 else None
        if got:
            codes, lds, bf16 = got
            descs = table
            table += _aligned((j - k) * C.sizeof(_lib.ConvDesc) // 4)
            op = prg.ConvChainOp(descs=prg.Ref("chain", descs), codes=prg.Ref("chain", table), n=j - k, B=ops[k].B,
                                 lds_bytes=lds, bf16=bf16, plan=tuple(codes), name=f"chain[{ops[k].name}..{ops[j - 1].name}]")
            table += _aligned(j - k)
            fused.append((op, k, j - k))
        elif cln_pair(k):
            a, b = ops[k], ops[k + 1]
            op = prg.ClnStepOp(x=a.x, stat_slope=a.slope, sums=a.sums, state=a.state, mr=a.mr, gain=b.gain, bias=b.bias,
                               slope=b.slope, add=b.add, out=b.out, B=b.B, T=b.T, P=b.P, C=b.C, mode=b.mode, eps=a.eps,
                               name=b.name + "_step")
            fused.append((op, k, 2))
            j = k + 2
        else:
            j = max(j, k + 1)
            fused += [(ops[t], t, 1) for t in range(k, j)]
        k = j
    return fused


def chain_planner(arr) -> Callable:
    lib = _lib.load()

    def plan(first: int, count: int):
        descs = (_lib.ConvDesc * count)(*[arr[first + t].conv for t in range(count)])
        codes = (C.c_int * count)()
        lds, bf16 = C.c_int(0), C.c_int(0)
        if lib.eab_conv_st_chain_plan(descs, count, codes, C.byref(lds), C.byref(bf16)) != 0:
            return None
        return list(codes), lds.value, bf16.value
    return plan


def chain_tables(arr, fused: Sequence) -> bytes:
    buf = bytearray()
    for op, first, count in fused:
        if op.kind == prg.OP_CONV_CHAIN:
            buf += bytes(4 * op.descs.off - len(buf)) + b"".join(bytes(arr[first + t].conv) for t in range(count))
            buf += bytes(4 * op.codes.off - len(buf)) + bytes((C.c_int * count)(*op.plan))
    return bytes(buf)


def graph_branches_allowed() -> bool:
    return os.environ.get("EAB_GRAPH_BRANCHES", "1") != "0"


class BoundProgram:
    BOUNDARY: tuple = ()

    def __init__(self, device: torch.device, arenas: Dict[str, torch.Tensor], lists: Dict[str, list],
                 lanes: Dict[str, list], sync: Dict[str, dict]):
        self.device, self.arenas = device, arenas
        self.lists, self.lanes, self.sync = lists, lanes, sync
        self.arrays = {name: (_lib.Op * len(ops))() for name, ops in lists.items()}
        self.window: dict = {}
        self._ptrs = None
        self.graphs: Optional[Dict[str, LaneGraphs]] = None
        self.graph_failed = False
        self.static: Dict[str, torch.Tensor] = {}
        self._direct: Dict[str, LaneGraphs] = {}

    def bind(self, *ptrs) -> bool:
        ptrs += (None,) * (len(self.BOUNDARY) - len(ptrs))
        if ptrs == self._ptrs:
            return False
        self._ptrs = ptrs
        bases = self.bases()
        for name, ops in self.lists.items():
            encode(ops, bases, out=self.arrays[name], **self.window)
        return True

    def bases(self) -> Dict[str, Optional[int]]:
        assert self._ptrs is not None, "bind the program first"
        bases = {k: t.data_ptr() for k, t in self.arenas.items()}
        bases.update(zip(self.BOUNDARY, self._ptrs))
        return bases

    def capture(self, *shapes) -> bool:
        if self.graphs is not None or self.graph_failed:
            return self.graphs is not None
        try:
            self.static = {k: torch.zeros(s, dtype=torch.float32, device=self.device)
                           for k, s in zip(self.BOUNDARY, shapes) if s is not None}
            self.bind(*(self.static[k].data_ptr() if k in self.static else None for k in self.BOUNDARY))
            side = torch.cuda.Stream(device=self.device)
            side.wait_stream(torch.cuda.current_stream())
            with torch.cuda.stream(side):
                for name, ops in self.lists.items():
                    self._launch(name, side.cuda_stream, 0, len(ops))
            torch.cuda.current_stream().wait_stream(side)
            graphs = {name: LaneGraphs(self.device, self._plan(name), functools.partial(self._launch, name))
                      for name in self.lists}
            for lg in graphs.values():
                lg.capture()
            self.graphs = graphs
        except Exception as e:
            warnings.warn(f"eabnet_amd: hipGraph capture failed ({e!r}); using direct launches")
            self.graphs, self.graph_failed, self._ptrs = None, True, None
        return self.graphs is not None

    def _plan(self, name: str) -> list:
        n = len(self.lists[name])
        sync = self.sync.get(name)
        return plan_segments(n, self.lanes[name], sync) if sync and graph_branches_allowed() else single_lane(n)

    def _launch(self, name: str, stream: int, first: int, n: int) -> None:
        ops = C.cast(C.byref(self.arrays[name], first * C.sizeof(_lib.Op)), C.POINTER(_lib.Op))
        _lib.check(_lib.load().eab_run_program(ops, n, C.c_void_p(stream)), f"eab_run_program({name})")

    def run(self, name: str, stream: int, first: int = 0, count: Optional[int] = None) -> None:
        if first == 0 and count is None and self.sync.get(name) and graph_branches_allowed():
            assert torch.cuda.current_stream().cuda_stream == stream, "multi-lane programs run on torch's current stream"
            if name not in self._direct:
                self._direct[name] = LaneGraphs(self.device, self._plan(name), functools.partial(self._launch, name))
            self._direct[name].run_direct()
            return
        self._launch(name, stream, first, len(self.lists[name]) - first if count is None else count)
```

### include/eabnet_hip.h

```cpp
#ifndef EABNET_HIP_H
#define EABNET_HIP_H

#include <stdint.h>

#ifdef __cplusplus
extern "C" {
#endif

#define EAB_ABI_VERSION 10

#define EAB_OK          0
#define EAB_EINVAL      1
#define EAB_EUNSUPPORTED 2
#define EAB_EHIP_BASE   1000

typedef void* eab_stream_t;

int         eab_abi_version(void);
const char* eab_error_string(int code);

typedef struct eab_time_window {
    const int32_t* pos;
    int32_t count;
    const int32_t* lens;
} eab_time_window;

#define EAB_STFT_LAYOUT_BTFM2 0
#define EAB_STFT_LAYOUT_B2TF  1
int eab_stft_compress_f32(const float* wav, const float* window, const float* twiddle,
                          float* out, int B, int M, int L, int n_fft, int hop,
                          int layout, eab_stream_t stream);

int eab_stft_compress_lens_f32(const float* wav, const float* window, const float* twiddle,
                               float* out, const int32_t* lens, int B, int M, int L_cap, int n_fft,
                               int hop, int layout, eab_stream_t stream);

int eab_stft_frames_f32(const float* wav, float* frames, int B, int M, int L, int n_fft, int hop,
                        eab_stream_t stream);

int eab_istft_f32(const float* spec, const float* window, const float* twiddle, float* wav, int B, int T,
                  int n_fft, int hop, eab_stream_t stream);

int eab_istft_lens_f32(const float* spec, const float* window, const float* twiddle, float* wav, const int32_t* lens,
                       int B, int T_cap, int n_fft, int hop, eab_stream_t stream);

#define EAB_ACT_SIGMOID 0
#define EAB_ACT_TANH    1
#define EAB_ACT_RELU    2
int eab_gag_pack_f32(const float* inpt, const float* pre_x, float* enc_in, float* pre, int B, int T, int F,
                     int ld, eab_time_window win, eab_stream_t stream);
int eab_gag_crm_f32(const float* pre, const float* g, const float* r, const float* i, float* pre_out,
                    float* planar, int B, int T, int F, int ld, int lin_ld, int act, eab_time_window win,
                    eab_stream_t stream);
int eab_gag_crm_bwd_f32(const float* pre, const float* g, const float* dplanar, const float* dpre_out, const float* acc_in,
                        float* dg, float* dr, float* di, float* dpre, int B, int T, int F, int ld, int lin_ld, int act,
                        eab_stream_t stream);

int eab_com_mag_mse_loss_f32(const float* esti, const float* label, const int32_t* frames, int B, int T, int F,
                             float* partial, int partial_blocks, float* loss, float* grad, eab_stream_t stream);

int eab_energy_ratios_f32(const float* est, long long est_stride, int est_cap, const float* clean, long long clean_stride,
                          int clean_cap, const float* noisy, long long noisy_stride, int noisy_cap, const int32_t* lens, int B,
                          double* partial, int partial_spans, double* out, eab_stream_t stream);
int eab_com_mag_mse_loss_lens_f32(const float* esti, const float* label, const int32_t* frames, int B, int T_esti, int T_label,
                                  int F, double* partial, int partial_spans, double* loss, eab_stream_t stream);

int eab_filter_sum_f32(const float* w, const float* x, float* y, int B, int T, int F, int M,
                       eab_stream_t stream);

#define EAB_MAX_TAPS 16

#define EAB_XF_NONE       0
#define EAB_XF_NORM_PRELU 1
#define EAB_XF_PRELU_NORM 2

#define EAB_EPI_LINEAR  0
#define EAB_EPI_GLU     1
#define EAB_EPI_RELU    2
#define EAB_EPI_MULSIG  3
#define EAB_EPI_ADD     4
#define EAB_EPI_DUALGATE 5
#define EAB_EPI_PHASE2  6

typedef struct eab_conv_desc {
    const float* src0;
    const float* src1;
    const float* xf0;
    const float* xf1;
    const float* slope0;
    const float* slope1;
    int32_t C0, C1;
    int32_t xf_mode;
    const float* w;
    const float* bias;
    int32_t N, Kpad;
    int32_t B, T, Fin, Fout;
    int32_t No;
    int32_t ostride, ophase, istride;
    int32_t ntaps;
    int32_t dt[EAB_MAX_TAPS];
    int32_t ioff[EAB_MAX_TAPS];
    int32_t epi;
    const float* aux;
    float* dst;
    float* dst_acc;
    int32_t Cout;
    float* stats;
    int32_t nsets;
    const float* stat_slope0;
    const float* stat_slope1;
    int32_t stat_tiles;
    int32_t stat_tile0;
    int32_t bm;
    const float* fin_stats;
    const float* fin_gamma0;
    const float* fin_beta0;
    const float* fin_gamma1;
    const float* fin_beta1;
    int32_t fin_tiles, fin_nsets, fin_count;
    float fin_eps;
    int32_t precision;
    int32_t korder;
    eab_time_window win;
    int32_t* fz_counter;
    const float* fz_gamma0;
    const float* fz_beta0;
    float* fz_xf0;
    const float* fz_gamma1;
    const float* fz_beta1;
    float* fz_xf1;
    float fz_eps;
    float* glu_dump;
    const float* ph1_w;
    int32_t ph1_No, ph1_ophase, ph1_ntaps, ph1_Kpad;
    int32_t ph1_dt[EAB_MAX_TAPS];
    int32_t ph1_ioff[EAB_MAX_TAPS];
    const float* f2_w;
    float* f2_dst;
    float* f2_stats;
    const float* f2_stat_slope0;
    const float* f2_stat_slope1;
    int32_t f2_N, f2_nsets, f2_stat_tiles;
    int32_t p2_mask1;
    int32_t src_bf16;
} eab_conv_desc;

#define EAB_PREC_F32   0
#define EAB_PREC_F16X3 1
#define EAB_PREC_BF16  2
#define EAB_KORDER_TAP   0
#define EAB_KORDER_CHUNK 1
#define EAB_KORDER_FRAG  2

int eab_conv_tiles(int T, int No, int bm);
int eab_conv_f32(const eab_conv_desc* d, eab_stream_t stream);
int eab_conv_bf16(const eab_conv_desc* d, eab_stream_t stream);

int eab_in_finalize_f32(const float* stats, int B, int C, int nsets, int stat_tiles,
                        int count , float eps,
                        const float* gamma0, const float* beta0, float* xf0,
                        const float* gamma1, const float* beta1, float* xf1,
                        eab_stream_t stream);

int eab_norm_act_f32(const float* a, const float* xfa, const float* slopea,
                     const float* b, const float* xfb, const float* slopeb,
                     float* out, int B, int P, int C, eab_stream_t stream);

int eab_lstm64_f32(const float* x, const float* ln_g, const float* ln_b, float ln_eps,
                   const float* wcat, const float* bias, float* h_out,
                   int B, int T, int F, eab_stream_t stream);
int eab_lstm64_prec_f32(const float* x, const float* ln_g, const float* ln_b, float ln_eps,
                        const float* wcat, const float* bias, float* h_out,
                        int B, int T, int F, int precision, eab_stream_t stream);
int eab_lstm64_bf16(const float* x, const float* ln_g, const float* ln_b, float ln_eps,
                    const float* wcat, const float* bias, float* h_out, int B, int T, int F, eab_stream_t stream);

int eab_bfw_filter_sum_f32(const float* y1, const float* w2, const float* b2, const float* x,
                           float* out, float* bfw, int B, int T, int F, int M,
                           eab_stream_t stream);

#define EAB_OP_CONV        1
#define EAB_OP_IN_FINALIZE 2
#define EAB_OP_NORM_ACT    3
#define EAB_OP_LSTM64      4
#define EAB_OP_BFW_FS      5
#define EAB_OP_MEMSET0     6
#define EAB_OP_GAG_PACK    7
#define EAB_OP_GAG_CRM     8
#define EAB_OP_CONV_CHAIN  9

typedef struct eab_wgrad_desc {
    const float* dz;
    const float* src0;
    const float* src1;
    float* dw;
    float* dbias;
    int32_t N, C0, C1, Kpad;
    int32_t B, T, Fin, Fz, No, ostride, ophase, istride;
    int32_t ntaps;
    int32_t dt[EAB_MAX_TAPS];
    int32_t ioff[EAB_MAX_TAPS];
    int32_t rows_per_wg;
    int32_t precision;
    int32_t bf16_mask;
} eab_wgrad_desc;

typedef struct eab_op {
    int32_t kind;
    int32_t i[8];
    float   f[2];
    const void* p[12];
    eab_time_window win;
    eab_conv_desc conv;
    eab_wgrad_desc wgrad;
} eab_op;
int eab_run_program(const eab_op* ops, int n_ops, eab_stream_t stream);

int eab_conv_st_chain_plan(const eab_conv_desc* descs, int n, int* codes, int* lds_bytes, int* bf16);
int eab_conv_st_chain_run(const eab_conv_desc* dev_descs, const int* dev_codes, int n, int B, int lds_bytes, int bf16,
                          eab_stream_t stream);

typedef struct eab_shift_desc {
    float* ptr;
    int32_t row_floats;
    int32_t rows;
} eab_shift_desc;
int eab_shift_rows_f32(const eab_shift_desc* dev_descs, int n, int B, int T, int src_pos, int H, eab_stream_t stream);

int eab_norm_act_win_f32(const float* a, const float* xfa, const float* slopea, const float* b,
                         const float* xfb, const float* slopeb, float* out, int B, int T, int rows_per_t, int C,
                         eab_time_window win, eab_stream_t stream);
int eab_lstm64_stream_f32(const float* x, const float* ln_g, const float* ln_b, float ln_eps, const float* wcat,
                          const float* bias, float* h_out, float* c_state, int B, int T, int F, int precision,
                          eab_time_window win, eab_stream_t stream);
int eab_bfw_filter_sum_win_f32(const float* y1, const float* w2, const float* b2, const float* x, float* out,
                               float* bfw, int B, int T, int F, int M, eab_time_window win, eab_stream_t stream);
int eab_zero_rows_f32(float* ptr, int B, int T, int row_floats, eab_time_window win, eab_stream_t stream);

int eab_mlp_bfw_filter_sum_f32(const float* h, const float* w1, const float* b1, const float* w2, const float* b2,
                               const float* x, float* out, float* bfw, int B, int T, int F, int M,
                               eab_time_window win, eab_stream_t stream);


int eab_gather_f32(const float* flat, const int32_t* ia, const int32_t* ib, float* out, long long n, eab_stream_t stream);

int eab_train_in_stats_f32(const float* x, const float* slope, int B, int P, int C, float eps, const float* gamma,
                           const float* beta, float* xf, float* mr, eab_stream_t stream);
int eab_train_in1d_f32(const float* x, const float* slope, int B, int P, int C, float eps, const float* gamma,
                       const float* beta, float* xf, float* mr, float* y, eab_stream_t stream);
int eab_train_in1d_multi_f32(const float* x, const float* slope, int B, int P, int C, int xC, float eps, const float* gamma,
                             const float* beta, float* xf, float* mr, float* y, eab_stream_t stream);
int eab_in_finalize_mr_f32(const float* stats, int B, int C, int nsets, int stat_tiles, int count, float eps,
                           const float* gamma0, const float* beta0, float* xf0, const float* gamma1,
                           const float* beta1, float* xf1, float* mr0, float* mr1, eab_stream_t stream);
int eab_train_norm_act_f32(const float* x, const float* xf, const float* slope, const float* add, float* y, int B, int P,
                           int C, int mode, eab_stream_t stream);
#define EAB_NB_SUMS_ZEROED 0x100
#define EAB_NB_SUM_COPIES 8
#define EAB_STORE_BF16 0x200
int eab_train_norm_bwd_f32(const float* dy, const float* x, const float* mr, const float* gamma, const float* beta,
                           const float* slope, float* sums, const float* acc_in, float* dx, float* dgamma, float* dbeta,
                           float* dslope, int B, int P, int C, int mode, eab_stream_t stream);
int eab_train_norm_bwd_multi_f32(const float* dy0, const float* dy1, const float* x, const float* mr, const float* gamma,
                                 const float* slope, float* sums, const float* acc_in, float* dx, float* dgamma, float* dbeta,
                                 float* dslope, int B, int P, int xC, eab_stream_t stream);
int eab_glu_bwd_f32(const float* dy, const float* dump, float* dz, long long rows, int N, eab_stream_t stream);
int eab_glu_bwd_ex_f32(const float* dy, const float* dump, float* dz, long long rows, int N, int flags, eab_stream_t stream);
int eab_gate_fwd_f32(const float* a, const float* r, float* z, long long n, eab_stream_t stream);
int eab_gate_bwd_f32(const float* dz, const float* a, const float* r, float* da, float* dr, long long n, eab_stream_t stream);
int eab_add_f32(const float* a, const float* b, float* out, long long n, eab_stream_t stream);
int eab_copy_f32(const float* src, float* dst, long long n, eab_stream_t stream);
int eab_relu_bwd_f32(const float* dy, const float* y, float* dx, long long n, eab_stream_t stream);
int eab_colsum_f32(const float* x, float* out, long long rows, int N, eab_stream_t stream);
int eab_filter_sum_ld_f32(const float* w, const float* x, float* y, int B, int T, int F, int M, int ld, eab_stream_t stream);
int eab_filter_sum_bwd_f32(const float* dout, const float* x, float* dw, int B, int T, int F, int M, int ld, eab_stream_t stream);
int eab_layernorm64_fwd_f32(const float* x, const float* g, const float* b, float eps, float* y, float* mr, long long rows,
                            eab_stream_t stream);
int eab_layernorm64_bwd_f32(const float* dy, const float* x, const float* mr, const float* g, float* dx, float* dg,
                            float* db, long long rows, eab_stream_t stream);
int eab_lstm64_train_fwd_f32(const float* x, const float* wcat, const float* bias, float* h_out, float* gates, int B, int T,
                             int F, eab_stream_t stream);
int eab_lstm64_bwd_f32(const float* gates, const float* dh_out, const float* wcat, float* dgates, int B, int T, int F,
                       eab_stream_t stream);
int eab_lstm64_train_fwd_prec_f32(const float* x, const float* wcat, const float* bias, float* h_out, float* gates, int B, int T,
                                  int F, int precision, eab_stream_t stream);
int eab_lstm64_bwd_prec_f32(const float* gates, const float* dh_out, const float* wcat, float* dgates, int B, int T, int F,
                            int precision, eab_stream_t stream);

int eab_wgrad_f32(const eab_wgrad_desc* d, eab_stream_t stream);
int eab_wgrad_batchable(const eab_wgrad_desc* descs, int n, int stride_bytes);
int eab_wgrad_batch_f32(const eab_wgrad_desc* descs, int n, int stride_bytes, eab_stream_t stream);

#define EAB_OP_GATHER      16
#define EAB_OP_IN_STATS    17
#define EAB_OP_TR_NORM_ACT 18
#define EAB_OP_NORM_BWD    19
#define EAB_OP_GLU_BWD     20
#define EAB_OP_GATE_FWD    21
#define EAB_OP_GATE_BWD    22
#define EAB_OP_ADD         23
#define EAB_OP_RELU_BWD    24
#define EAB_OP_COLSUM      25
#define EAB_OP_FILTER_SUM  26
#define EAB_OP_FS_BWD      27
#define EAB_OP_LN_FWD      28
#define EAB_OP_LN_BWD      29
#define EAB_OP_LSTM_TRAIN  30
#define EAB_OP_LSTM_BWD    31
#define EAB_OP_WGRAD       32

int eab_cln_stats_f32(const float* x, const float* slope, int B, int T, int P, int C, float eps, double* sums, double* state,
                      float* mr, eab_time_window win, eab_stream_t stream);
int eab_train_cln_bwd_f32(const float* dy, const float* x, const float* mr, const float* gain, const float* bias,
                          const float* slope, double* rowsums, float* ab, float* part, const float* acc_in, float* dx,
                          int B, int T, int P, int C, int mode, eab_stream_t stream);
int eab_cln_apply_f32(const float* x, const float* mr, const float* gain, const float* bias, const float* slope,
                      const float* add, float* y, int B, int T, int P, int C, int mode, eab_time_window win,
                      eab_stream_t stream);
int eab_gate_rows_f32(const float* a, const float* r, float* z, int B, int T, int row_floats, eab_time_window win,
                      eab_stream_t stream);
int eab_cln_step_f32(const float* x, const float* stat_slope, double* sums, double* state, float* mr, const float* gain,
                     const float* bias, const float* slope, const float* add, float* y, int B, int T, int P, int C, int mode,
                     float eps, eab_time_window win, eab_stream_t stream);
#define EAB_OP_CLN_STATS 33
#define EAB_OP_CLN_APPLY 34
#define EAB_OP_GATE_ROWS 35
#define EAB_OP_GAG_CRM_BWD 36
#define EAB_OP_CLN_STEP 38
#define EAB_OP_CLN_BWD 37

int eab_sizeof_conv_desc(void);
int eab_sizeof_op(void);
int eab_sizeof_wgrad_desc(void);

#ifdef __cplusplus
}
#endif
#endif
```

Measured before the change: 984,400 frames/s.

## Fold norm+PReLU pass into the LSTM input load when it is the sole reader

Adds an XIN template path to all LSTM64 kernels (f32, q, h3) that applies the per-channel instance-norm scale/shift and PReLU to x as it is loaded. A runtime pass fuses a NormAct op with the next LSTM op when the LSTM is the only consumer, so the normalized activation is never written to or re-read from global memory, and one launch is dropped. This costs a few extra VALU ops per loaded element in the recurrent loop. The intermediate activation then no longer exists, so fusion only applies when taps are not kept, and it can be disabled by environment variable.

```diff
diff --git a/eabnet_amd/_lib.py b/eabnet_amd/_lib.py
--- a/eabnet_amd/_lib.py
+++ b/eabnet_amd/_lib.py
@@ -83,6 +83,8 @@
     "eab_norm_act_win_f32": (C.c_int, [C.c_void_p] * 7 + [C.c_int] * 4 + [TimeWindow, C.c_void_p]),
     "eab_lstm64_stream_f32": (C.c_int, [C.c_void_p] * 3 + [C.c_float] + [C.c_void_p] * 4 + [C.c_int] * 4
                               + [TimeWindow, C.c_void_p]),
+    "eab_lstm64_xin_f32": (C.c_int, [C.c_void_p] * 5 + [C.c_float] + [C.c_void_p] * 4 + [C.c_int] * 4 + [TimeWindow, C.c_void_p]),
+    "eab_lstm64_xin_seq16_f32": (C.c_int, [C.c_void_p] * 5 + [C.c_float] + [C.c_void_p] * 4 + [C.c_int] * 4 + [TimeWindow, C.c_void_p]),
     "eab_bfw_filter_sum_win_f32": (C.c_int, [C.c_void_p] * 6 + [C.c_int] * 4 + [TimeWindow, C.c_void_p]),
     "eab_mlp_bfw_filter_sum_f32": (C.c_int, [C.c_void_p] * 8 + [C.c_int] * 4 + [TimeWindow, C.c_void_p]),
     "eab_zero_rows_f32": (C.c_int, [C.c_void_p] + [C.c_int] * 3 + [TimeWindow, C.c_void_p]),
diff --git a/eabnet_amd/csrc/lstm.hip b/eabnet_amd/csrc/lstm.hip
--- a/eabnet_amd/csrc/lstm.hip
+++ b/eabnet_amd/csrc/lstm.hip
@@ -23,14 +23,16 @@
 typedef unsigned int u32x4 __attribute__((ext_vector_type(4)));
 #define LS_OOB 0x80000000u
 
-template <bool LN, bool DUMP>
+template <bool LN, bool DUMP, bool XIN = false>
 __global__ __launch_bounds__(256) void lstm64_kernel(const float* __restrict__ x, const float* __restrict__ ln_g,
                                                      const float* __restrict__ ln_b, float ln_eps,
                                                      const float* __restrict__ wcat, const float* __restrict__ bias,
                                                      float* __restrict__ h_out, int T, int F, int S,
                                                      const int* __restrict__ t_pos, int t_count,
                                                      float* __restrict__ c_state, float* __restrict__ gates,
-                                                     const int* __restrict__ lens = nullptr) {
+                                                     const int* __restrict__ lens = nullptr,
+                                                     const float* __restrict__ xin_xf = nullptr,
+                                                     const float* __restrict__ xin_slope = nullptr) {
     __shared__ __attribute__((aligned(16))) float xs[2][LS_SEQ * LS_LD];
     __shared__ __attribute__((aligned(16))) float hs[2][LS_SEQ * LS_LD];
     const int tid = threadIdx.x, lane = tid & 63, wave = tid >> 6;
@@ -72,12 +74,26 @@
         g4 = *reinterpret_cast<const f32x4*>(ln_g + lc);
         b4 = *reinterpret_cast<const f32x4*>(ln_b + lc);
     }
+    f32x4 xs01 = {1.f, 0.f, 1.f, 0.f}, xs23 = {1.f, 0.f, 1.f, 0.f}, xsl = {1.f, 1.f, 1.f, 1.f};
+    if (XIN) {
+        const float* xp = xin_xf + ((size_t)sb * LS_H + lc) * 2;
+        xs01 = *reinterpret_cast<const f32x4*>(xp);
+        xs23 = *reinterpret_cast<const f32x4*>(xp + 4);
+        xsl = *reinterpret_cast<const f32x4*>(xin_slope + lc);
+    }
 
     auto load_x = [&](int t) -> f32x4 {
         const unsigned off = (sv && t < t_hi) ? seq_off + (unsigned)t * t_stride : LS_OOB;
         return __builtin_bit_cast(f32x4, __builtin_amdgcn_raw_buffer_load_b128(rx, off, 0, 0));
     };
-    auto norm_store = [&](f32x4 v, int buf) {
+    auto norm_store = [&](f32x4 v, int buf, int t) {
+        if (XIN) {
+            const bool live = sv && t < t_hi;
+            v[0] = live ? eab_prelu(fmaf(v[0], xs01[0], xs01[1]), xsl[0]) : 0.0f;
+            v[1] = live ? eab_prelu(fmaf(v[1], xs01[2], xs01[3]), xsl[1]) : 0.0f;
+            v[2] = live ? eab_prelu(fmaf(v[2], xs23[0], xs23[1]), xsl[2]) : 0.0f;
+            v[3] = live ? eab_prelu(fmaf(v[3], xs23[2], xs23[3]), xsl[3]) : 0.0f;
+        }
         if (LN) {
             const float mean = ls_row_sum((v[0] + v[1]) + (v[2] + v[3])) * (1.0f / 64.0f);
             f32x4 dlt = {v[0] - mean, v[1] - mean, v[2] - mean, v[3] - mean};
@@ -108,8 +124,8 @@
 
     *reinterpret_cast<f32x4*>(&hs[0][ls * LS_LD + lc]) = __builtin_bit_cast(
         f32x4, __builtin_amdgcn_raw_buffer_load_b128(rh, (sv && t_lo > 0) ? seq_off + (unsigned)(t_lo - 1) * t_stride : LS_OOB, 0, 0));
-    norm_store(load_x(t_lo), 0);
-    norm_store(load_x(t_lo + 1), 1);
+    norm_store(load_x(t_lo), 0, t_lo);
+    norm_store(load_x(t_lo + 1), 1, t_lo + 1);
     const int u = wave * 16 + ln;
     float cst[4] = {0.f, 0.f, 0.f, 0.f};
     if (c_state && t_lo > 0) {
@@ -135,13 +151,13 @@
 #pragma unroll
         for (int g = 0; g < 4; ++g) acc[g] = accx[g];
         mma(hf, wh, acc, I0{}, I4{});
-        norm_store(xq, cur);
+        norm_store(xq, cur, t + 2);
         frags(xs[nxt], xf);
         if (LN) {
 #pragma unroll
             for (int i = 0; i < 16; ++i) {
                 __builtin_amdgcn_sched_group_barrier(0x008, 4, 0);
-                __builtin_amdgcn_sched_group_barrier(0x002, 6, 0);
+                __builtin_amdgcn_sched_group_barrier(0x002, XIN ? 7 : 6, 0);
             }
         }
         __builtin_amdgcn_sched_barrier(0);
@@ -211,14 +227,16 @@
     }
 }
 
-template <bool LN, int G, bool DUMP = false>
+template <bool LN, int G, bool DUMP = false, bool XIN = false>
 __global__ __launch_bounds__(256) void lstm64_q_kernel(const float* __restrict__ x, const float* __restrict__ ln_g,
                                                        const float* __restrict__ ln_b, float ln_eps,
                                                        const float* __restrict__ wcat, const float* __restrict__ bias,
                                                        float* __restrict__ h_out, int T, int F, int S,
                                                        const int* __restrict__ t_pos, int t_count,
                                                        float* __restrict__ c_state, float* __restrict__ gates = nullptr,
-                                                       const int* __restrict__ lens = nullptr) {
+                                                       const int* __restrict__ lens = nullptr,
+                                                       const float* __restrict__ xin_xf = nullptr,
+                                                       const float* __restrict__ xin_slope = nullptr) {
     constexpr int NSEQ = 4 * G;
     constexpr int NCH = G == 1 ? 8 : (G == 2 ? 4 : 2);
     __shared__ __attribute__((aligned(16))) float xs[2][NSEQ * LS_LD];
@@ -259,11 +277,25 @@
         g4 = *reinterpret_cast<const f32x4*>(ln_g + lc);
         b4 = *reinterpret_cast<const f32x4*>(ln_b + lc);
     }
+    f32x4 xs01 = {1.f, 0.f, 1.f, 0.f}, xs23 = {1.f, 0.f, 1.f, 0.f}, xsl = {1.f, 1.f, 1.f, 1.f};
+    if (XIN) {
+        const float* xp = xin_xf + ((size_t)sb * LS_H + lc) * 2;
+        xs01 = *reinterpret_cast<const f32x4*>(xp);
+        xs23 = *reinterpret_cast<const f32x4*>(xp + 4);
+        xsl = *reinterpret_cast<const f32x4*>(xin_slope + lc);
+    }
     auto load_x = [&](int t) -> f32x4 {
         const unsigned off = (sv && t < t_hi) ? seq_off + (unsigned)t * t_stride : LS_OOB;
         return __builtin_bit_cast(f32x4, __builtin_amdgcn_raw_buffer_load_b128(rx, off, 0, 0));
     };
-    auto norm_store = [&](f32x4 v, int buf) {
+    auto norm_store = [&](f32x4 v, int buf, int t) {
+        if (XIN) {
+            const bool live = sv && t < t_hi;
+            v[0] = live ? eab_prelu(fmaf(v[0], xs01[0], xs01[1]), xsl[0]) : 0.0f;
+            v[1] = live ? eab_prelu(fmaf(v[1], xs01[2], xs01[3]), xsl[1]) : 0.0f;
+            v[2] = live ? eab_prelu(fmaf(v[2], xs23[0], xs23[1]), xsl[2]) : 0.0f;
+            v[3] = live ? eab_prelu(fmaf(v[3], xs23[2], xs23[3]), xsl[3]) : 0.0f;
+        }
         if (LN) {
             const float mean = ls_row_sum((v[0] + v[1]) + (v[2] + v[3])) * (1.0f / 64.0f);
             f32x4 dlt = {v[0] - mean, v[1] - mean, v[2] - mean, v[3] - mean};
@@ -281,7 +313,7 @@
     if (ls < NSEQ)
         *reinterpret_cast<f32x4*>(&hs[0][ls * LS_LD + lc]) = __builtin_bit_cast(
             f32x4, __builtin_amdgcn_raw_buffer_load_b128(rh, (sv && t_lo > 0) ? seq_off + (unsigned)(t_lo - 1) * t_stride : LS_OOB, 0, 0));
-    norm_store(load_x(t_lo), 0);
+    norm_store(load_x(t_lo), 0, t_lo);
     float cst[G][4];
 #pragma unroll
     for (int q = 0; q < G; ++q)
@@ -329,7 +361,7 @@
             __builtin_amdgcn_sched_group_barrier(0x008, 24, 0);
             __builtin_amdgcn_sched_barrier(0);
         }
-        norm_store(xq, nxt);
+        norm_store(xq, nxt, t + 1);
 #pragma unroll
         for (int q = 0; q < G; ++q) {
             f32x4 pre = acc[q][0];
@@ -375,18 +407,21 @@
 template <int G>
 static void lstm64_q_launch(bool ln, int grid, hipStream_t st, const float* x, const float* ln_g, const float* ln_b,
                             float ln_eps, const float* wcat, const float* bias, float* h_out, int T, int F, int S,
-                            const int* t_pos, int t_count, float* cs, const int* lens) {
-    if (ln)
-        hipLaunchKernelGGL((lstm64_q_kernel<true, G>), dim3(grid), dim3(256), 0, st, x, ln_g, ln_b, ln_eps, wcat, bias,
-                           h_out, T, F, S, t_pos, t_count, cs, nullptr, lens);
-    else
-        hipLaunchKernelGGL((lstm64_q_kernel<false, G>), dim3(grid), dim3(256), 0, st, x, ln_g, ln_b, ln_eps, wcat, bias,
-                           h_out, T, F, S, t_pos, t_count, cs, nullptr, lens);
+                            const int* t_pos, int t_count, float* cs, const int* lens, const float* xin_xf, const float* xin_slope) {
+#define LQ_GO(LN_, XIN_)                                                                                                   \
+    hipLaunchKernelGGL((lstm64_q_kernel<LN_, G, false, XIN_>), dim3(grid), dim3(256), 0, st, x, ln_g, ln_b, ln_eps, wcat, bias, \
+                       h_out, T, F, S, t_pos, t_count, cs, nullptr, lens, xin_xf, xin_slope)
+    if (xin_xf) {
+        if (ln) LQ_GO(true, true); else LQ_GO(false, true);
+    } else {
+        if (ln) LQ_GO(true, false); else LQ_GO(false, false);
+    }
+#undef LQ_GO
 }
 
 int eab_lstm64_h3_launch(const float* x, const float* ln_g, const float* ln_b, float ln_eps, const float* wcat,
                          const float* bias, float* h_out, int T, int F, int S, int precision, const int* t_pos, int t_count,
-                         float* c_state, const int* lens, hipStream_t stream);
+                         float* c_state, const int* lens, const float* xin_xf, const float* xin_slope, hipStream_t stream);
 
 extern "C" int eab_lstm64_f32(const float* x, const float* ln_g, const float* ln_b, float ln_eps, const float* wcat,
                               const float* bias, float* h_out, int B, int T, int F, eab_stream_t stream) {
@@ -403,29 +438,53 @@
 extern "C" int eab_lstm64_stream_f32(const float* x, const float* ln_g, const float* ln_b, float ln_eps,
                                      const float* wcat, const float* bias, float* h_out, float* c_state, int B, int T,
                                      int F, int precision, eab_time_window win, eab_stream_t stream) {
+    return eab_lstm64_xin_f32(x, nullptr, nullptr, ln_g, ln_b, ln_eps, wcat, bias, h_out, c_state, B, T, F, precision, win, stream);
+}
+
+static int lstm64_xin_run(const float* x, const float* xin_xf, const float* xin_slope, const float* ln_g, const float* ln_b,
+                          float ln_eps, const float* wcat, const float* bias, float* h_out, float* c_state, int B, int T, int F,
+                          int precision, eab_time_window win, eab_stream_t stream, bool seq16) {
     EAB_CHECK_ARG(x && wcat && bias && h_out && B > 0 && T > 0 && F > 0);
     EAB_CHECK_ARG(win.pos == nullptr || (win.count > 0 && c_state));
     EAB_CHECK_ARG(precision == EAB_PREC_F32 || precision == EAB_PREC_F16X3 || precision == EAB_PREC_BF16);
     EAB_CHECK_ARG((ln_g == nullptr) == (ln_b == nullptr));
+    EAB_CHECK_ARG((xin_xf == nullptr) == (xin_slope == nullptr));
+    EAB_CHECK_ARG(!xin_xf || ((((uintptr_t)xin_xf | (uintptr_t)xin_slope) & 15) == 0));
     const long long S = (long long)B * F;
     EAB_CHECK_ARG(S * T * LS_H * 4 < (1ll << 31));
     float* cs = win.pos ? c_state : nullptr;
     if (precision != EAB_PREC_F32)
         return eab_lstm64_h3_launch(x, ln_g, ln_b, ln_eps, wcat, bias, h_out, T, F, (int)S, precision, win.pos, win.count, cs,
-                                    win.lens, eab_stream(stream));
-    if (S <= 2048) {
+                                    win.lens, xin_xf, xin_slope, eab_stream(stream));
+    if (S <= 2048 && !seq16) {
         lstm64_q_launch<1>(ln_g != nullptr, (int)((S + 3) / 4), eab_stream(stream), x, ln_g, ln_b, ln_eps, wcat, bias, h_out,
-                           T, F, (int)S, win.pos, win.count, cs, win.lens);
+                           T, F, (int)S, win.pos, win.count, cs, win.lens, xin_xf, xin_slope);
         EAB_RETURN_LAUNCH_STATUS();
     }
     const int grid = (int)((S + LS_SEQ - 1) / LS_SEQ);
-    if (ln_g)
-        hipLaunchKernelGGL((lstm64_kernel<true, false>), dim3(grid), dim3(256), 0, eab_stream(stream), x, ln_g, ln_b, ln_eps,
-                           wcat, bias, h_out, T, F, (int)S, win.pos, win.count, cs, nullptr, win.lens);
-    else
-        hipLaunchKernelGGL((lstm64_kernel<false, false>), dim3(grid), dim3(256), 0, eab_stream(stream), x, ln_g, ln_b, ln_eps,
-                           wcat, bias, h_out, T, F, (int)S, win.pos, win.count, cs, nullptr, win.lens);
+#define LS_GO(LN_, XIN_)                                                                                                    \
+    hipLaunchKernelGGL((lstm64_kernel<LN_, false, XIN_>), dim3(grid), dim3(256), 0, eab_stream(stream), x, ln_g, ln_b, ln_eps, \
+                       wcat, bias, h_out, T, F, (int)S, win.pos, win.count, cs, nullptr, win.lens, xin_xf, xin_slope)
+    if (xin_xf) {
+        if (ln_g) LS_GO(true, true); else LS_GO(false, true);
+    } else {
+        if (ln_g) LS_GO(true, false); else LS_GO(false, false);
+    }
+#undef LS_GO
     EAB_RETURN_LAUNCH_STATUS();
+}
+
+extern "C" int eab_lstm64_xin_f32(const float* x, const float* xin_xf, const float* xin_slope, const float* ln_g,
+                                  const float* ln_b, float ln_eps, const float* wcat, const float* bias, float* h_out,
+                                  float* c_state, int B, int T, int F, int precision, eab_time_window win, eab_stream_t stream) {
+    return lstm64_xin_run(x, xin_xf, xin_slope, ln_g, ln_b, ln_eps, wcat, bias, h_out, c_state, B, T, F, precision, win, stream, false);
+}
+
+extern "C" int eab_lstm64_xin_seq16_f32(const float* x, const float* xin_xf, const float* xin_slope, const float* ln_g,
+                                        const float* ln_b, float ln_eps, const float* wcat, const float* bias, float* h_out,
+                                        float* c_state, int B, int T, int F, int precision, eab_time_window win,
+                                        eab_stream_t stream) {
+    return lstm64_xin_run(x, xin_xf, xin_slope, ln_g, ln_b, ln_eps, wcat, bias, h_out, c_state, B, T, F, precision, win, stream, true);
 }
 
 int eab_lstm64_bf_train_launch(const float* x, const float* wcat, const float* bias, float* h_out, float* gates, int T, int F, int S,
diff --git a/eabnet_amd/csrc/lstm_h3.hip b/eabnet_amd/csrc/lstm_h3.hip
--- a/eabnet_amd/csrc/lstm_h3.hip
+++ b/eabnet_amd/csrc/lstm_h3.hip
@@ -46,13 +46,15 @@
     return (float)__builtin_bit_cast(_Float16, hi) + (float)__builtin_bit_cast(_Float16, lo);
 }
 
-template <bool LN, bool BF, bool DUMP = false, int NS = LH_SEQ>
+template <bool LN, bool BF, bool DUMP = false, int NS = LH_SEQ, bool XIN = false>
 __global__ __launch_bounds__(256) void lstm64_h3_kernel(const float* __restrict__ x, const float* __restrict__ ln_g,
                                                         const float* __restrict__ ln_b, float ln_eps,
                                                         const float* __restrict__ wcat, const float* __restrict__ bias,
                                                         float* __restrict__ h_out, int T, int F, int S,
                                                         const int* __restrict__ t_pos, int t_count, float* __restrict__ c_state,
-                                                        float* __restrict__ gates = nullptr, const int* __restrict__ lens = nullptr) {
+                                                        float* __restrict__ gates = nullptr, const int* __restrict__ lens = nullptr,
+                                                        const float* __restrict__ xin_xf = nullptr,
+                                                        const float* __restrict__ xin_slope = nullptr) {
     using v8 = std::conditional_t<BF, bf16x8, h16x8>;
     using e16 = std::conditional_t<BF, __bf16, _Float16>;
     __shared__ __attribute__((aligned(16))) char xs[2][LH_SEQ * LH_ROW];
@@ -104,13 +106,27 @@
         g4 = *reinterpret_cast<const f32x4*>(ln_g + lc);
         b4 = *reinterpret_cast<const f32x4*>(ln_b + lc);
     }
+    f32x4 xs01 = {1.f, 0.f, 1.f, 0.f}, xs23 = {1.f, 0.f, 1.f, 0.f}, xsl = {1.f, 1.f, 1.f, 1.f};
+    if (XIN) {
+        const float* xp = xin_xf + ((size_t)sb * 64 + lc) * 2;
+        xs01 = *reinterpret_cast<const f32x4*>(xp);
+        xs23 = *reinterpret_cast<const f32x4*>(xp + 4);
+        xsl = *reinterpret_cast<const f32x4*>(xin_slope + lc);
+    }
     const int lrow = ls * LH_ROW + (lc >> 5) * 128 + (lc & 31) * 2;
 
     auto load_x = [&](int t) -> f32x4 {
         const unsigned off = (sv && t < t_hi) ? seq_off + (unsigned)t * t_stride : LH_OOB;
         return __builtin_bit_cast(f32x4, __builtin_amdgcn_raw_buffer_load_b128(rx, off, 0, 0));
     };
-    auto norm_store = [&](f32x4 v, int buf) {
+    auto norm_store = [&](f32x4 v, int buf, int t) {
+        if (XIN) {
+            const bool live = sv && t < t_hi;
+            v[0] = live ? eab_prelu(fmaf(v[0], xs01[0], xs01[1]), xsl[0]) : 0.0f;
+            v[1] = live ? eab_prelu(fmaf(v[1], xs01[2], xs01[3]), xsl[1]) : 0.0f;
+            v[2] = live ? eab_prelu(fmaf(v[2], xs23[0], xs23[1]), xsl[2]) : 0.0f;
+            v[3] = live ? eab_prelu(fmaf(v[3], xs23[2], xs23[3]), xsl[3]) : 0.0f;
+        }
         if (LN) {
             const float mean = lh_row_sum((v[0] + v[1]) + (v[2] + v[3])) * (1.0f / 64.0f);
             f32x4 dlt = {v[0] - mean, v[1] - mean, v[2] - mean, v[3] - mean};
@@ -159,8 +175,8 @@
         *reinterpret_cast<uint2*>(&hs[0][lrow]) = make_uint2(h01, h23);
         *reinterpret_cast<uint2*>(&hs[0][lrow + 64]) = make_uint2(l01, l23);
     }
-    norm_store(load_x(t_lo), 0);
-    norm_store(load_x(t_lo + 1), 1);
+    norm_store(load_x(t_lo), 0, t_lo);
+    norm_store(load_x(t_lo + 1), 1, t_lo + 1);
     const int uq = wave * 16 + ln;
     float cst[4] = {0.f, 0.f, 0.f, 0.f};
     if (c_state && t_lo > 0) {
@@ -205,7 +221,7 @@
         for (int g = 0; g < 4; ++g) acc[g] = accx[g];
         mma(hh, hl, whh, whl, acc);
         frags(xs[nxt], xh, xl);
-        norm_store(xq, cur);
+        norm_store(xq, cur, t + 2);
         __builtin_amdgcn_sched_barrier(0);
         char* hrow = &hs[nxt][hcol];
 #pragma unroll
@@ -272,16 +288,23 @@
 
 int eab_lstm64_h3_launch(const float* x, const float* ln_g, const float* ln_b, float ln_eps, const float* wcat,
                          const float* bias, float* h_out, int T, int F, int S, int precision, const int* t_pos, int t_count,
-                         float* c_state, const int* lens, hipStream_t stream) {
+                         float* c_state, const int* lens, const float* xin_xf, const float* xin_slope, hipStream_t stream) {
     const int grid = (S + LH_SEQ - 1) / LH_SEQ;
-#define LH_GO(LN_, BF_)                                                                                                     \
-    hipLaunchKernelGGL((lstm64_h3_kernel<LN_, BF_>), dim3(grid), dim3(256), 0, stream, x, ln_g, ln_b, ln_eps, wcat, bias, h_out, \
-                       T, F, S, t_pos, t_count, c_state, nullptr, lens)
+#define LH_GO(LN_, BF_, XIN_)                                                                                               \
+    hipLaunchKernelGGL((lstm64_h3_kernel<LN_, BF_, false, LH_SEQ, XIN_>), dim3(grid), dim3(256), 0, stream, x, ln_g, ln_b, ln_eps, \
+                       wcat, bias, h_out, T, F, S, t_pos, t_count, c_state, nullptr, lens, xin_xf, xin_slope)
+#define LH_PICK(BF_)                                                              \
+    if (xin_xf) {                                                                 \
+        if (ln_g) LH_GO(true, BF_, true); else LH_GO(false, BF_, true);          \
+    } else {                                                                      \
+        if (ln_g) LH_GO(true, BF_, false); else LH_GO(false, BF_, false);        \
+    }
     if (precision == EAB_PREC_BF16) {
-        if (ln_g) LH_GO(true, true); else LH_GO(false, true);
+        LH_PICK(true)
     } else {
-        if (ln_g) LH_GO(true, false); else LH_GO(false, false);
-    }
+        LH_PICK(false)
+    }
+#undef LH_PICK
 #undef LH_GO
     EAB_RETURN_LAUNCH_STATUS();
 }
diff --git a/eabnet_amd/csrc/program.hip b/eabnet_amd/csrc/program.hip
--- a/eabnet_amd/csrc/program.hip
+++ b/eabnet_amd/csrc/program.hip
@@ -100,9 +100,9 @@
                                           (float*)o.p[6], o.i[0], o.i[1], o.i[2], stream);
                 break;
             case EAB_OP_LSTM64:
-                rc = eab_lstm64_stream_f32((const float*)o.p[0], (const float*)o.p[1], (const float*)o.p[2], o.f[0],
-                                           (const float*)o.p[3], (const float*)o.p[4], (float*)o.p[5], (float*)o.p[6],
-                                           o.i[0], o.i[1], o.i[2], o.i[3], o.win, stream);
+                rc = eab_lstm64_xin_f32((const float*)o.p[0], (const float*)o.p[7], (const float*)o.p[8], (const float*)o.p[1],
+                                        (const float*)o.p[2], o.f[0], (const float*)o.p[3], (const float*)o.p[4], (float*)o.p[5],
+                                        (float*)o.p[6], o.i[0], o.i[1], o.i[2], o.i[3], o.win, stream);
                 break;
             case EAB_OP_BFW_FS:
                 rc = eab_mlp_bfw_filter_sum_f32((const float*)o.p[0], (const float*)o.p[6], (const float*)o.p[7],
diff --git a/eabnet_amd/model.py b/eabnet_amd/model.py
--- a/eabnet_amd/model.py
+++ b/eabnet_amd/model.py
@@ -13,7 +13,7 @@
 from . import _lib
 from . import program as prg
 from .graphs import LaneGraphs
-from .runtime import BoundProgram, chain_planner, chain_tables, encode, fuse_step
+from .runtime import BoundProgram, chain_planner, chain_tables, encode, fuse_single_reader, fuse_step
 from .runtime import graph_branches_allowed
 from .spec import GagConfig, NetConfig, ParamSpec, gag_param_specs, param_specs
 
@@ -62,8 +62,9 @@
 class _Bound(BoundProgram):
     BOUNDARY = ("in", "out", "in2")
 
-    def __init__(self, prog: prg.Program, device: torch.device):
+    def __init__(self, prog: prg.Program, device: torch.device, keep_taps: bool = True):
         self.prog = prog
+        self.keep_taps = keep_taps
         self.weights = torch.from_numpy(prog.weights).to(device)
         self.acts = torch.empty(max(prog.act_floats, 1), dtype=torch.float32, device=device)
         super().__init__(device, {"w": self.weights, "a": self.acts}, {"run": prog.ops}, {"run": prog.lanes}, {"run": prog.sync})
@@ -74,6 +75,7 @@
         self.window = {"t_pos": self.t_pos.data_ptr() if prog.chunk else None, "chunk": prog.chunk,
                        "lens": self.lens.data_ptr() if prog.varlen else None}
         self.fused, self.exec_ops = None, None
+        self.unwritten: list = []
         self._carry_dev = None
 
     def reset_counters(self) -> None:
@@ -104,6 +106,13 @@
         self._carry_dev = None
         p = self.prog
         if not p.chunk:
+            self.fused, self.exec_ops, self.unwritten = None, None, []
+            if not self.keep_taps and os.environ.get("EAB_FUSE_SINGLE_READER", "1") != "0":
+                fused = fuse_single_reader(p.ops)
+                if len(fused) < len(p.ops):
+                    self.fused = fused
+                    self.exec_ops = encode([op for op, _, _ in fused], self.bases(), **self.window)
+                    self.unwritten = [p.ops[first].out for _, first, count in fused if count == 2]
             return True
         self.fused, self.exec_ops = None, None
         self.arenas.pop("chain", None)
@@ -165,6 +174,10 @@
         p = self.prog
         n = p.B * p.T * act.F * act.C
         assert act.ref.arena == "a"
+        if act.ref in self.unwritten:
+            raise ValueError("this activation is not in memory: the bound run folds its norm + PReLU pass into the LSTM that reads "
+                             "it (runtime.fuse_single_reader); bind with keep_taps=True (the modules: dump_bfw = True) or set "
+                             "EAB_FUSE_SINGLE_READER=0")
         return self.acts[act.ref.off:act.ref.off + n].view(p.B, p.T, act.F, act.C)
 
 
@@ -268,7 +281,7 @@
                 while cache and (len(cache) >= limit or sum(4 * b.acts.numel() for b in cache.values()) + need > budget):
                     old, _ = cache.popitem(last=False)
                     versions.pop(old, None)
-                bound = cache[key] = _Bound(prog, device)
+                bound = cache[key] = _Bound(prog, device, keep_taps=self.dump_bfw)
             else:
                 bound.update_weights(prog.weights)
             versions[key] = fp
diff --git a/eabnet_amd/program.py b/eabnet_amd/program.py
--- a/eabnet_amd/program.py
+++ b/eabnet_amd/program.py
@@ -186,6 +186,8 @@
     win: bool = False
     name: str = ""
     kind: int = OP_LSTM64
+    xin_xf: Optional[Ref] = None
+    xin_slope: Optional[Ref] = None
 
 
 @dataclass
diff --git a/eabnet_amd/runtime.py b/eabnet_amd/runtime.py
--- a/eabnet_amd/runtime.py
+++ b/eabnet_amd/runtime.py
@@ -26,7 +26,8 @@
     prg.FinalizeOp: (("B", "C", "nsets", "stat_tiles", "count"),
                      ("stats", "gamma0", "beta0", "xf0", "gamma1", "beta1", "xf1", "mr0"), ("eps",)),
     prg.NormActOp: (("B", "P", "C", "T"), ("a", "xfa", "slopea", "b", "xfb", "slopeb", "out"), ()),
-    prg.LstmOp: (("B", "T", "F", "precision"), ("x", "ln_g", "ln_b", "wcat", "bias", "h_out", "c_state"), ("ln_eps",)),
+    prg.LstmOp: (("B", "T", "F", "precision"), ("x", "ln_g", "ln_b", "wcat", "bias", "h_out", "c_state", "xin_xf", "xin_slope"),
+                 ("ln_eps",)),
     prg.BfwOp: (("B", "T", "F", "M"), ("y1", "w2", "b2", "x", "out", "bfw", "w1", "b1"), ()),
     prg.MemsetOp: ((None, None, "B", "T", "row"), ("ptr",), ()),
     prg.ClnStatsOp: (("B", "T", "P", "C"), ("x", "slope", "sums", "state", "mr"), ("eps",)),
@@ -145,6 +146,29 @@
     return fused
 
 
+def _refs_read(op) -> list:
+    import dataclasses
+    if not dataclasses.is_dataclass(op):
+        return [r for r in getattr(op, "p", []) if isinstance(r, prg.Ref)]
+    return [v for v in (getattr(op, f.name) for f in dataclasses.fields(op)) if isinstance(v, prg.Ref)]
+
+
+def fuse_single_reader(ops: Sequence) -> List[Tuple[object, int, int]]:
+    import dataclasses
+    fused, k, n = [], 0, len(ops)
+    while k < n:
+        a, b = ops[k], ops[k + 1] if k + 1 < n else None
+        if (a.kind == prg.OP_NORM_ACT and a.b is None and b is not None and b.kind == prg.OP_LSTM64 and b.x == a.out
+                and b.xin_xf is None and a.C == 64 and (a.B, a.P) == (b.B, b.T * b.F) and a.win == b.win
+                and not any(a.out in _refs_read(o) for j, o in enumerate(ops) if j not in (k, k + 1))):
+            fused.append((dataclasses.replace(b, x=a.a, xin_xf=a.xfa, xin_slope=a.slopea, name=f"{a.name}+{b.name}"), k, 2))
+            k += 2
+        else:
+            fused.append((a, k, 1))
+            k += 1
+    return fused
+
+
 def chain_planner(arr) -> Callable:
     lib = _lib.load()
 
diff --git a/include/eabnet_hip.h b/include/eabnet_hip.h
--- a/include/eabnet_hip.h
+++ b/include/eabnet_hip.h
@@ -233,6 +233,12 @@
 int eab_lstm64_stream_f32(const float* x, const float* ln_g, const float* ln_b, float ln_eps, const float* wcat,
                           const float* bias, float* h_out, float* c_state, int B, int T, int F, int precision,
                           eab_time_window win, eab_stream_t stream);
+int eab_lstm64_xin_f32(const float* x, const float* xin_xf, const float* xin_slope, const float* ln_g, const float* ln_b,
+                       float ln_eps, const float* wcat, const float* bias, float* h_out, float* c_state, int B, int T, int F,
+                       int precision, eab_time_window win, eab_stream_t stream);
+int eab_lstm64_xin_seq16_f32(const float* x, const float* xin_xf, const float* xin_slope, const float* ln_g, const float* ln_b,
+                             float ln_eps, const float* wcat, const float* bias, float* h_out, float* c_state, int B, int T,
+                             int F, int precision, eab_time_window win, eab_stream_t stream);
 int eab_bfw_filter_sum_win_f32(const float* y1, const float* w2, const float* b2, const float* x, float* out,
                                float* bfw, int B, int T, int F, int M, eab_time_window win, eab_stream_t stream);
 int eab_zero_rows_f32(float* ptr, int B, int T, int row_floats, eab_time_window win, eab_stream_t stream);
```

After: 997,800 frames/s (median of 6 runs). +1.4%, better.
